# pansanity666/TransHuman

Hardware: AMD Instinct MI355X
Metric: rays/sec (512x512, 64 samples/ray) (higher is better)
Workload: dtype f32 (fp16 hi/lo x3 MFMA emulation)

## Files before the change

### include/transhuman_hip.h

```cpp
#ifndef TRANSHUMAN_HIP_H
#define TRANSHUMAN_HIP_H

#include <stddef.h>
#include <stdint.h>

#ifdef __cplusplus
extern "C" {
#endif

#define TH_ABI_VERSION 12

typedef struct th_ctx th_ctx;
typedef void* th_stream;

int         th_abi_version(void);
const char* th_last_error(void);
int         th_ctx_create(int device, th_ctx** out);
void        th_ctx_destroy(th_ctx* ctx);
size_t      th_sizeof(const char* type_name);

enum { TH_PROF_HULL = 0, TH_PROF_DPARF = 1, TH_PROF_GATHER = 2, TH_PROF_MLP = 3, TH_PROF_COMPOSITE = 4,
       TH_PROF_VIT = 5, TH_PROF_FOLD = 6 , TH_PROF_PHASES = 8 };
int th_profile_enable(th_ctx* ctx, int on);
int th_profile_read(th_ctx* ctx, double* ms_out, int64_t* count_out);
int th_host_wait_read(th_ctx* ctx, double* ms_out);
int th_clock_probe(th_ctx* ctx, int64_t* out_dev , th_stream stream);
int th_fused_cycles(th_ctx* ctx, int64_t* counters_dev);

typedef struct {
    const float* w;
    const float* b;
    int out_f;
    int in_f;
} th_linear;

typedef struct {
    th_linear fc_0, alpha_res_0;
    th_linear key0, val0;
    th_linear key1, val1;
    th_linear fc_1, fc_2, fc_3, alpha_fc;
    th_linear feature_fc, rgb_res_0, view_fc, rgb_res_1, fc_4, rgb_fc;
    th_linear upsample_color;
} th_mlp_weights;

typedef struct {
    const float *ln1_w, *ln1_b, *ln2_w, *ln2_b;
    th_linear qkv, proj, fc1, fc2;
} th_vit_block;

int th_set_mlp_weights(th_ctx* ctx, const th_mlp_weights* w, th_stream stream);
int th_set_mlp_mode(th_ctx* ctx, int mode);
int th_set_fused_waves(th_ctx* ctx, int waves);
int th_set_tok_gather(th_ctx* ctx, int on);
int th_set_tex_rows(th_ctx* ctx, int on);

#define TH_RANGE_SLOTS 8
#define TH_RANGE_FP16_LIMIT 0x7B53u
#define TH_RANGE_FP16_FLOOR 0x2400u
int th_set_vit_mode(th_ctx* ctx, int mode);
int th_range_snapshot(th_ctx* ctx, th_stream stream);
int th_range_read(th_ctx* ctx, int slot, uint32_t* out );
int th_range_last_slot(th_ctx* ctx);
int th_set_chunk_samples(int n);
int th_set_vit_weights(th_ctx* ctx, int depth, int dim, int heads, const th_vit_block* blocks,
                       const float* norm_w, const float* norm_b, th_stream stream);

size_t th_linear_workspace_bytes(int out_f, int in_f);
int th_linear_forward(th_ctx* ctx, const float* A, int lda, int M, const th_linear* lin, int act,
                      float* C, int ldc, void* workspace, size_t workspace_bytes, th_stream stream);

typedef struct {
    const float* pts;
    const float* ray_o;
    const float* ray_d;
    const float* near;
    const float* far;
    const float* t_vals;
    const float* one_minus_t;
    int R, S;
    const float* z_vals;
    const float* sigma_noise;
} th_points;

size_t th_hull_workspace_bytes(int n_verts);
int th_hull_mask(th_ctx* ctx, const th_points* p, const float* verts_world, int n_verts, float thresh,
                 uint8_t* mask_out, int32_t* ray_hit_out, void* workspace, size_t workspace_bytes,
                 th_stream stream);

int th_paint_group(th_ctx* ctx, const float* holder_map_nchw, int V, int C, int H, int W,
                   const float* verts_world, int n_verts, const float* cams, const float* scale_xy,
                   const uint8_t* vizmap, const int32_t* csr_offsets, const int32_t* csr_members,
                   int n_clusters, float* painted_out , float* tokens_out,
                   th_stream stream);
int th_segment_mean_f32(th_ctx* ctx, const float* src, int width, const int32_t* csr_offsets,
                        const int32_t* csr_members, int n_clusters, float* out, th_stream stream);
int th_segment_mean_rot_f64(th_ctx* ctx, const double* blend, const int32_t* csr_offsets,
                            const int32_t* csr_members, int n_clusters, float* rot_out,
                            th_stream stream);

#define TH_MAP_FULL    384
#define TH_MAP_COMPACT 260
#define TH_MAP_SPLIT   256

int th_upsample_concat_nhwc(th_ctx* ctx, const float* img, const float* lat0, const float* lat1,
                            const float* lat2, const int32_t* dims_host, int V, int H, int W,
                            const float* color_w, const float* color_b, float* out_nhwc, th_stream stream);
int th_upsample_concat_split(th_ctx* ctx, const float* img, const float* lat0, const float* lat1, const float* lat2,
                             const int32_t* dims_host, int V, int H, int W, float* out, th_stream stream);
int th_map_box(th_ctx* ctx, const float* verts_a, int na, const float* verts_b, int nb, const float* cams, int V,
               const float* scale_xy, int H, int W, float reach, int32_t* box_out, th_stream stream);
int th_upsample_concat_split_box(th_ctx* ctx, const float* img, const float* lat0, const float* lat1, const float* lat2,
                                 const int32_t* dims_host, int V, int H, int W, float* out, const int32_t* box,
                                 th_stream stream);
size_t th_map_demand_bytes(int V, int H, int W);
int th_upsample_concat_split_demand(th_ctx* ctx, const float* img, const float* lat0, const float* lat1, const float* lat2,
                                    const int32_t* dims_host, int V, int H, int W, float* out, const int32_t* box,
                                    const void* demand, th_stream stream);
size_t th_paint_group_nhwc_workspace_bytes(int V, int n_verts, int C, int out_f);
int th_paint_group_nhwc(th_ctx* ctx, const float* map_nhwc, int V, int H, int W, int C,
                        const float* verts_world, int n_verts, const float* cams, const float* scale_xy,
                        const uint8_t* vizmap, const th_linear* reduction, const th_linear* color_lift,
                        const int32_t* csr_offsets,
                        const int32_t* csr_members, int n_clusters, float* tokens_out, void* workspace,
                        size_t workspace_bytes, th_stream stream);

size_t th_conv_pack_bytes(int cout, int cin, int ks);
int th_conv_pack(th_ctx* ctx, const float* w, int cout, int cin, int ks, void* packed, size_t packed_bytes,
                 float* inv_scale_out, th_stream stream);
int th_conv2d_supported(int cin, int cout, int ks, int stride);
int th_conv2d(th_ctx* ctx, const float* x, int N, int cin, int H, int W, const void* packed, float inv_scale, int cout,
              int ks, int stride, float* y, th_stream stream);

int th_maxpool3x3s2(th_ctx* ctx, const float* x, int planes, int H, int W, float* y, th_stream stream);

size_t th_bn_workspace_bytes(int N, int C, int HW);
// ... 70 lines not shown
size_t th_ssim_workspace_bytes(int h, int w, int c);
int th_ssim(th_ctx* ctx, const float* a, const float* b, int h, int w, int c, int pitch, double* out, void* workspace,
            size_t workspace_bytes, th_stream stream);

size_t th_lpips_pack_bytes(void);
int th_lpips_pack(th_ctx* ctx, const float* const* conv_w , const float* const* conv_b ,
                  const float* const* lin_w , void* packed, size_t bytes, th_stream stream);
size_t th_lpips_workspace_bytes(int n, int h, int w);
int th_lpips(th_ctx* ctx, const float* in0, const float* in1, int n, int h, int w, const void* packed, double* out,
             void* workspace, size_t workspace_bytes, th_stream stream);

size_t th_rasterize_workspace_bytes(int V, int n_verts, int n_faces, int H, int W);
int th_rasterize_mesh(th_ctx* ctx, const float* verts_world, int n_verts, const int32_t* faces, int n_faces, const float* cams,
                      int V, int H, int W, float background, float* depth, int32_t* pix_to_face, void* workspace,
                      size_t workspace_bytes, th_stream stream);
int th_vertex_visibility(th_ctx* ctx, const int32_t* pix_to_face, const int32_t* faces, int n_faces, int n_verts, int V, int H,
                         int W, uint8_t* vis, th_stream stream);
int th_depth_visibility(th_ctx* ctx, const float* verts_world, int n_verts, const float* cams, int V, const float* depthmaps,
                        int H, int W, float det, float* surface_depth, uint8_t* vis_mask, float* relative_depth,
                        th_stream stream);

size_t th_vertex_normals_workspace_bytes(int n_verts, int n_faces);
int th_vertex_normals(th_ctx* ctx, const float* verts, int n_verts, const int32_t* faces, int n_faces, int flip, float* normals,
                      int32_t* status, void* workspace, size_t workspace_bytes, th_stream stream);
int th_shade_mesh(th_ctx* ctx, const float* verts_world, const float* vertex_normals, int n_verts, const int32_t* faces,
                  int n_faces, const float* cams, int V, int H, int W, const int32_t* pix_to_face, const float* light_host ,
                  const float* background_host , float ambient, float diffuse, float specular, int shininess, float* image,
                  th_stream stream);

int th_prep_views(th_ctx* ctx, const uint8_t* img_u8, const uint8_t* msk_u8, int V, int H0, int W0, const float* K ,
                  const float* D , int n, int mask_bkgd, int white_bkgd, const float* lut , float* out_img,
                  uint8_t* out_msk, th_stream stream);
int th_prep_mask(th_ctx* ctx, const uint8_t* a, const uint8_t* b_or_null, int V, int H0, int W0, int border, uint8_t* out,
                 th_stream stream);

typedef struct {
    const double* v_template;
    const double* shapedirs;
    const double* posedirs;
    const double* J_regressor;
    const double* weights;
    const int32_t* parent;
    int n_verts;
} th_smpl_model;
size_t th_smpl_workspace_bytes(int n_verts);
int th_smpl_lbs(th_ctx* ctx, const th_smpl_model* model, const float* pose_aa, const float* rot, const double* beta,
                double* verts, double* joints, double* T, void* workspace, size_t workspace_bytes,
                th_stream stream);

int th_view_embed(th_ctx* ctx, const float* ray_d, int R, int view_res, float* out, th_stream stream);

typedef struct {
    const int32_t* box;
    float          reach;
    const float*   img;
    const float*   lat0;
    const float*   lat1;
    const float*   lat2;
    int32_t        dims[6];
    const void*    demand;
} th_map_source;

typedef struct {
    const float* verts_world;
    int          n_verts;
    const float* Rh;
    const float* Th;
    const float* cams;
    const float* scale_xy;
    const float* pixel_map_nhwc;
    int          V, H, W;
    int          map_channels;
    const float* tokens;
    const float* centres;
    const float* rot;
    int          n_clusters;
    float        hull_thresh;
    int          small_frame_rays;
    const th_map_source* map_source;
    const float* map_fold;
} th_frame;

size_t th_render_workspace_bytes(const th_frame* f, int R, int S);
size_t th_shade_pool_bytes(th_ctx* ctx, const th_frame* f, long long n_valid, int with_pregather);
int th_render_rays(th_ctx* ctx, const th_frame* f, const th_points* rays, float* rgb, float* acc,
                   float* depth, int white_bkgd, void* workspace, size_t workspace_bytes,
                   void* shade_pool, size_t shade_pool_bytes, int64_t* stats_host, th_stream stream);

int th_render_prepass(th_ctx* ctx, const th_frame* f, const th_points* rays, void* workspace,
                      size_t workspace_bytes, th_stream stream);
int th_render_pregather(th_ctx* ctx, const th_frame* f, const th_points* rays, void* workspace,
                        size_t workspace_bytes, void* shade_pool, size_t shade_pool_bytes, th_stream stream);
int th_render_pregrid(th_ctx* ctx, const th_frame* f, const th_points* rays, void* workspace, size_t workspace_bytes,
                      th_stream stream);
int th_render_predemand(th_ctx* ctx, const th_frame* f, const th_points* rays, void* workspace, size_t workspace_bytes,
                        const float* verts_paint, int n_paint, void* demand, size_t demand_bytes, th_stream stream);
int th_render_pregather_early(th_ctx* ctx, const th_frame* f, const th_points* rays, void* workspace,
                              size_t workspace_bytes, void* shade_pool, size_t shade_pool_bytes, th_stream stream);
int th_render_prepass_wait(th_ctx* ctx, const void* workspace, int64_t* counts_host );
int th_render_prepass_cancel(th_ctx* ctx);
int th_render_prepass_drop(th_ctx* ctx, const void* workspace);

size_t th_sigma_grid_workspace_bytes(const th_frame* f, int P);
int th_eval_sigma_grid(th_ctx* ctx, const th_frame* f, const float* pts, int P, float* sigma_out,
                       void* workspace, size_t workspace_bytes, void* shade_pool, size_t shade_pool_bytes,
                       int64_t* stats_host, th_stream stream);

#ifdef __cplusplus
}
#endif
#endif
```

### transhuman_amd/csrc/k_mlp_fused8_kernel.h

```cpp
#pragma once
#include "k_mlp_fused_kernel.h"

typedef float f8_f4 __attribute__((ext_vector_type(4)));
typedef short f8_s4 __attribute__((ext_vector_type(4)));
typedef short f8_s8 __attribute__((ext_vector_type(8)));

#define F8_THREADS 512
#define F8_PART_FLOATS (3 * 8 * 32)
#define F8_PSTR 12
#define F8_MISC_FLOATS (F8_PSTR * 32 + F8_PART_FLOATS + 32 + 8)
#define F8_LDS_BYTES (ABUF_BYTES + MBUF_BYTES + F8_MISC_FLOATS * 4)
static_assert(F8_LDS_BYTES <= 163840, "the 8-wave tile must fit the CU's LDS");

#define F8_MFMA(A, B, C) __builtin_amdgcn_mfma_f32_16x16x32_f16((A), (B), (C), 0, 0, 0)

template <int CT>
__device__ __forceinline__ void f8_load_w(const uint4* __restrict__ wl, int t, uint4 (&w)[CT][2]) {
    const uint4* p = wl + (long long)t * (CT * 2 * 64);
#pragma unroll
    for (int c = 0; c < CT; ++c) {
        w[c][0] = p[(c * 2 + 0) * 64];
        w[c][1] = p[(c * 2 + 1) * 64];
    }
}
#define F8_WSLICE(L, wave, ct) ((L).w + (long long)(wave) * (L).KB * ((ct) * 2 * 64))

template <int NR, int ROWSTEP, bool PERM>
__device__ __forceinline__ void f8_load_x(const char* __restrict__ ahi, const char* __restrict__ alo, int aoff, int t,
                                          h8 (&xh)[NR], h8 (&xl)[NR]) {
    const int ko = (PERM ? 32 : 64) * t;
#pragma unroll
    for (int r = 0; r < NR; ++r) {
        xh[r] = *reinterpret_cast<const h8*>(ahi + r * ROWSTEP + aoff + ko);
        xl[r] = *reinterpret_cast<const h8*>(alo + r * ROWSTEP + aoff + ko);
    }
}
template <bool PERM>
__device__ __forceinline__ int f8_aoff(int lane, int str) {
    const int l = lane & 15, g = lane >> 4;
    return PERM ? l * str + 16 * (g >> 1) + 256 * (g & 1) : l * str + 16 * g;
}

template <int CT, int RT, int NR, int R0, bool FIRST>
__device__ __forceinline__ void f8_mfma_half(const uint4 (&w)[CT][2], const h8 (&xh)[NR], const h8 (&xl)[NR], f8_f4 (&acc)[CT][RT]) {
    const f8_f4 zero = {0.f, 0.f, 0.f, 0.f};
#pragma unroll
    for (int c = 0; c < CT; ++c)
#pragma unroll
        for (int r = 0; r < NR; ++r)
            acc[c][R0 + r] = F8_MFMA(*reinterpret_cast<const h8*>(&w[c][1]), xh[r], FIRST ? zero : acc[c][R0 + r]);
#pragma unroll
    for (int c = 0; c < CT; ++c)
#pragma unroll
        for (int r = 0; r < NR; ++r) acc[c][R0 + r] = F8_MFMA(*reinterpret_cast<const h8*>(&w[c][0]), xl[r], acc[c][R0 + r]);
#pragma unroll
    for (int c = 0; c < CT; ++c)
#pragma unroll
        for (int r = 0; r < NR; ++r) acc[c][R0 + r] = F8_MFMA(*reinterpret_cast<const h8*>(&w[c][0]), xh[r], acc[c][R0 + r]);
}

template <int NMEM, int NMF>
__device__ __forceinline__ void f8_interleave() {
    constexpr int NP = NMEM < NMF ? NMEM : NMF;
#pragma unroll
    for (int q = 0; q < NP; ++q) {
        __builtin_amdgcn_sched_group_barrier(0x008, 1, 0);
        __builtin_amdgcn_sched_group_barrier(0x120, 1, 0);
    }
    if constexpr (NMF > NP) __builtin_amdgcn_sched_group_barrier(0x008, NMF - NP, 0);
    if constexpr (NMEM > NP) __builtin_amdgcn_sched_group_barrier(0x120, NMEM - NP, 0);
    FM_SB();
}

template <int RT, int CT, int ROWSTEP, bool PERM, bool PRE = false>
__device__ __forceinline__ void f8_gemm(const char* __restrict__ ahi, const char* __restrict__ alo, int str,
                                        const uint4* __restrict__ wp, int T, int lane, f8_f4 (&acc)[CT][RT], uint4 (&w)[2][CT][2]) {
    static_assert(RT % 2 == 0, "row tiles come in halves");
    constexpr int NR = RT / 2;
    const uint4* wl = wp + lane;
    const int aoff = f8_aoff<PERM>(lane, str);
    h8 xah[NR], xal[NR], xbh[NR], xbl[NR];
    if (!PRE) f8_load_w<CT>(wl, 0, w[0]);
    f8_load_x<NR, ROWSTEP, PERM>(ahi, alo, aoff, 0, xah, xal);
    FM_SB();
    auto step = [&](auto first, auto par, int t) __attribute__((always_inline)) {
        constexpr bool F = decltype(first)::value;
        constexpr int PB = decltype(par)::value;
        const int tn = t + 1 < T ? t + 1 : T - 1;
        f8_load_x<NR, ROWSTEP, PERM>(ahi + NR * ROWSTEP, alo + NR * ROWSTEP, aoff, t, xbh, xbl);
        f8_load_w<CT>(wl, tn, w[PB ^ 1]);
        f8_mfma_half<CT, RT, NR, 0, F>(w[PB], xah, xal, acc);
        f8_interleave<2 * NR + 2 * CT, 3 * CT * NR>();
        f8_load_x<NR, ROWSTEP, PERM>(ahi, alo, aoff, tn, xah, xal);
        f8_mfma_half<CT, RT, NR, NR, F>(w[PB], xbh, xbl, acc);
        f8_interleave<2 * NR, 3 * CT * NR>();
    };
    step(std::true_type{}, std::integral_constant<int, 0>{}, 0);
    if (T > 1) {
        step(std::false_type{}, std::integral_constant<int, 1>{}, 1);
#pragma unroll 1
        for (int t = 2; t < T; t += 2) {
            step(std::false_type{}, std::integral_constant<int, 0>{}, t);
            step(std::false_type{}, std::integral_constant<int, 1>{}, t + 1);
        }
    }
}

template <int RT, int CT, int ROWSTEP, bool PERM, bool PRE = false>
__device__ __forceinline__ void f8_gemm3(const char* __restrict__ ahi, const char* __restrict__ alo, int str,
                                         const uint4* __restrict__ wp, int T, int lane, f8_f4 (&acc)[CT][RT], uint4 (&w)[2][CT][2]) {
    static_assert(RT % 3 == 0, "row tiles come in thirds");
    constexpr int NR = RT / 3;
    const uint4* wl = wp + lane;
    const int aoff = f8_aoff<PERM>(lane, str);
    h8 xh[2][NR], xl[2][NR];
    if (!PRE) f8_load_w<CT>(wl, 0, w[0]);
    f8_load_x<NR, ROWSTEP, PERM>(ahi, alo, aoff, 0, xh[0], xl[0]);
    FM_SB();
    auto sub = [&](auto first, auto sidx, int t) __attribute__((always_inline)) {
        constexpr int S = decltype(sidx)::value, G = S % 3, PB = S / 3, CUR = S & 1;
        constexpr bool F = decltype(first)::value && S < 3;
        constexpr int GN = (G + 1) % 3;
        const int tt = t + PB;
        const int tx = G == 2 ? (tt + 1 < T ? tt + 1 : T - 1) : tt;
        f8_load_x<NR, ROWSTEP, PERM>(ahi + GN * NR * ROWSTEP, alo + GN * NR * ROWSTEP, aoff, tx, xh[CUR ^ 1], xl[CUR ^ 1]);
        if constexpr (G == 0) f8_load_w<CT>(wl, tt + 1 < T ? tt + 1 : T - 1, w[PB ^ 1]);
        f8_mfma_half<CT, RT, NR, G * NR, F>(w[PB], xh[CUR], xl[CUR], acc);
        f8_interleave<2 * NR + (G == 0 ? 2 * CT : 0), 3 * CT * NR>();
    };
    auto pair = [&](auto first, int t) __attribute__((always_inline)) {
        sub(first, std::integral_constant<int, 0>{}, t); sub(first, std::integral_constant<int, 1>{}, t);
        sub(first, std::integral_constant<int, 2>{}, t); sub(first, std::integral_constant<int, 3>{}, t);
        sub(first, std::integral_constant<int, 4>{}, t); sub(first, std::integral_constant<int, 5>{}, t);
    };
    pair(std::true_type{}, 0);
#pragma unroll 1
    for (int t = 2; t < T; t += 2) pair(std::false_type{}, t);
}
template <int RT, int CT, int ROWSTEP, bool PERM, bool PRE = false>
__device__ __forceinline__ void f8_gemm_rt(const char* __restrict__ ahi, const char* __restrict__ alo, int str,
                                           const uint4* __restrict__ wp, int T, int lane, f8_f4 (&acc)[CT][RT], uint4 (&w)[2][CT][2]) {
    if constexpr (RT % 3 == 0) f8_gemm3<RT, CT, ROWSTEP, PERM, PRE>(ahi, alo, str, wp, T, lane, acc, w);
    else f8_gemm<RT, CT, ROWSTEP, PERM, PRE>(ahi, alo, str, wp, T, lane, acc, w);
}

template <int STR, bool NONNEG = true>
__device__ __forceinline__ void f8_store_h(const f8_f4& t, int row, int col0, char* __restrict__ hi, char* __restrict__ lo, int lane,
                                           unsigned& rm) {
    const int c = col0 + 4 * (lane >> 4);
    uint2 a, b;
    split_pair(t[0], t[1], a.x, b.x);
    split_pair(t[2], t[3], a.y, b.y);
    range_acc<NONNEG>(rm, a.x);
    range_acc<NONNEG>(rm, a.y);
    *reinterpret_cast<uint2*>(hi + row * STR + 2 * c) = a;
    *reinterpret_cast<uint2*>(lo + row * STR + 2 * c) = b;
}
__device__ __forceinline__ f8_f4 f8_finish(const f8_f4& a, const float4& b, float inv_scale, bool relu) {
    const f32x2 sc = {inv_scale, inv_scale};
    f32x2 y01 = __builtin_elementwise_fma((f32x2){a[0], a[1]}, sc, (f32x2){b.x, b.y});
    f32x2 y23 = __builtin_elementwise_fma((f32x2){a[2], a[3]}, sc, (f32x2){b.z, b.w});
    if (relu) {
        y01 = __builtin_elementwise_max(y01, (f32x2){0.f, 0.f});
        y23 = __builtin_elementwise_max(y23, (f32x2){0.f, 0.f});
    }
    return (f8_f4){y01[0], y01[1], y23[0], y23[1]};
}
__device__ __forceinline__ float f8_xor(float v, int lane, int mask) {
    return __builtin_bit_cast(float, __builtin_amdgcn_ds_bpermute((lane ^ mask) << 2, __builtin_bit_cast(int, v)));
}
__device__ __forceinline__ float4 f8_bias(const float* __restrict__ bias, int col0, int lane) {
    return *reinterpret_cast<const float4*>(bias + col0 + 4 * (lane >> 4));
}

template <int RT, int NV, int H, int R0, bool FIRST>
__device__ __forceinline__ void f8_mfma_dual(const uint4 (&r3)[2][2], const uint4 (&ra)[1][2], const h8 (&mh)[1], const h8 (&ml)[1],
                                             const h8 (&xh)[NV], const h8 (&xl)[NV], f8_f4 (&a3)[2][2], f8_f4 (&va)[1][RT]) {
    const f8_f4 zero = {0.f, 0.f, 0.f, 0.f};
#pragma unroll
    for (int t = 0; t < 3; ++t) {
        const int wp = t == 0 ? 1 : 0;
        const bool lo = t == 1;
        const bool first = FIRST && t == 0;
        a3[0][H] = F8_MFMA(*reinterpret_cast<const h8*>(&r3[0][wp]), lo ? ml[0] : mh[0], first ? zero : a3[0][H]);
#pragma unroll
        for (int r = 0; r < NV; ++r) {
            va[0][R0 + r] = F8_MFMA(*reinterpret_cast<const h8*>(&ra[0][wp]), lo ? xl[r] : xh[r], first ? zero : va[0][R0 + r]);
            if (r == 0) a3[1][H] = F8_MFMA(*reinterpret_cast<const h8*>(&r3[1][wp]), lo ? ml[0] : mh[0], first ? zero : a3[1][H]);
        }
    }
}

template <int V>
__global__ __launch_bounds__(F8_THREADS, 2) void mlp_fused8_kernel(FusedParams P_arg) {
#define PK P_arg
    struct F8Dbg { long long* dbg; };
    const F8Dbg P{PK.dbg};
    extern __shared__ __attribute__((aligned(16))) char lds[];
    char* abuf = lds;
    char* mbuf = lds + ABUF_BYTES;
    float* misc = reinterpret_cast<float*>(lds + ABUF_BYTES + MBUF_BYTES);
    float* probs = misc;
    float* part = misc + F8_PSTR * 32;
    float* sig = part + F8_PART_FLOATS;
    int* flag = reinterpret_cast<int*>(sig + 32);

    const int tid = threadIdx.x, lane = tid & 63, wave = tid >> 6;
    const int l15 = lane & 15, g4 = lane >> 4;
    const int tile = (int)((blockIdx.x & 7) * (gridDim.x >> 3) + (blockIdx.x >> 3));
    const int pbase = tile * FM_PTS;
    if (pbase >= PK.P) return;
    const int npts = min(FM_PTS, PK.P - pbase);
    const int fm_dbg_tile = tile;
    const int zoff = 0;
    constexpr int ROWS = 32 * V, RT = 2 * V;
    constexpr int RS256 = 16 * STR256;
    int dbg_i = 1;
    long long dbg_t = 0;
    long long* dbg_keep = reinterpret_cast<long long*>(flag + 2);
    constexpr float inv_v = 1.0f / (float)V;
    unsigned rmax = 0u;
    unsigned seen_s = 0u, seen_p = 0u, seen_n = 0u, seen_i = 0u, seen_4 = 0u;
    char* a256_lo = abuf + ROWS * STR256;

    struct TexPre { unsigned h0, h1; fm_u4 rq; };
    auto tex_fetch = [&]() __attribute__((always_inline)) {
        int tl = tile;
        asm volatile("" : "+s"(tl));
        TexPre t;
        const unsigned* hb = PK.tex_hdr + (long long)tl * 512;
        t.h0 = hb[lane];
        t.h1 = hb[64 + lane];
        t.rq = (fm_u4){0u, 0u, 0u, 0u};
        if (tid < 64 * V) t.rq = *reinterpret_cast<const fm_u4*>(PK.tex_rec + (long long)tl * V * 32 * 8 + tid * 4);
        return t;
    };
    auto fill_tex = [&](const TexPre& pre, auto rgb, auto&& under) __attribute__((always_inline)) {
        constexpr bool RGB = decltype(rgb)::value;
        constexpr int TSTR = 1040, TMAX = 103, NK = (TMAX + 7) / 8, NR = 4 * V;
        static_assert(TMAX * TSTR <= ABUF_BYTES, "a pass of texel rows must fit the operand buffer");
        int wv = __builtin_amdgcn_readfirstlane(wave), tl = tile;
        asm volatile("" : "+s"(wv), "+s"(tl));
        const unsigned* hb = PK.tex_hdr + (long long)tl * 512;
        unsigned h0 = pre.h0, h1 = pre.h1;
        const int npass = __builtin_amdgcn_readfirstlane((int)(h0 >> 16));
        char* recl = reinterpret_cast<char*>(misc);
        static_assert(32 * V * 32 <= (F8_PSTR * 32 + F8_PART_FLOATS) * 4, "row records must fit probs + part");
        unsigned fv[NR][4] = {};
        f32x2 bias_lo = {0.f, 0.f}, bias_hi = {0.f, 0.f};
        if constexpr (!RGB) {
            const float4 b4 = *reinterpret_cast<const float4*>(PK.ar0.bias + 4 * lane);
            bias_lo = (f32x2){b4.x, b4.y};
            bias_hi = (f32x2){b4.z, b4.w};
        }
        for (int p = 0; p < npass; ++p) {
            if (p > 0) {
                FM_SYNCL();
                h0 = hb[p * 128 + lane];
                h1 = hb[p * 128 + 64 + lane];
            }
            const int U = __builtin_amdgcn_readfirstlane((int)(h0 & 0xffffu));
            {
                constexpr int NA = 7, NB = 10;
                const char* mbase = reinterpret_cast<const char*>(RGB ? PK.tex_map2 : PK.tex_map);
                const unsigned loff = (unsigned)lane * 16u;
                const int last = U - 1;
                fm_u4 ta[NA], tb[NB - NA], tc[NK - NB];
#pragma unroll
                for (int k = 0; k < NA; ++k) {
                    const int i = min(wv + 8 * k, last);
                    const unsigned id = (unsigned)__builtin_amdgcn_readlane((int)h0, 8 + i);
                    ta[k] = *reinterpret_cast<const fm_u4*>(mbase + TX_ADDR(id));
                }
                const bool more = U > 8 * NA, most = U > 8 * NB;
                if (more) {
#pragma unroll
// ... 175 lines not shown
            if (u0 > 0) {
                FM_SYNCL();
                if (tid < 2 * 32 * STRVD / 16) reinterpret_cast<uint4*>(wsp_hi)[tid] = make_uint4(zq, zq, zq, zq);
            }
            for (int u = wv; u < nU; u += 8) {
                const int cu = slot_centre(u0 + u);
                const char* g = reinterpret_cast<const char*>(PK.tsplit) + (long long)cu * 1024 + lane * 16;
#pragma unroll
                for (int vw = 0; vw < V; ++vw)
                    __builtin_amdgcn_global_load_lds((fm_gptr)(g + (long long)vw * PK.t_nc * 1024),
                                                     (fm_lptr)(abuf + (vw * 32 + u) * STOK_STR), 16, 0, 0);
            }
            FM_SYNCL();
            if (slot >= u0 && slot < u0 + 32) {
                _Float16 hi, lo;
                split_h(nw, hi, lo);
                *reinterpret_cast<_Float16*>(wsp_hi + ns * STRVD + 2 * (slot - u0)) = hi;
                *reinterpret_cast<_Float16*>(wsp_lo + ns * STRVD + 2 * (slot - u0)) = lo;
            }
            if (u0 == 0) {
#pragma unroll
                for (int t = 0; t < 2; ++t) {
                    h8 xh[2], xl[2];
                    f8_load_x<2, 16 * STR64, false>(pe_hi, pe_lo, aoffp, t, xh, xl);
                    if (t == 0) f8_mfma_half<2, 2, 2, 0, true>(wq[0], xh, xl, a1);
                    else f8_mfma_half<2, 2, 2, 0, false>(wq[1], xh, xl, a1);
                }
            }
            FM_SYNC();
            {
                h8 xh[2], xl[2];
                f8_load_x<2, 16 * STRVD, false>(wsp_hi, wsp_lo, aoffw, 0, xh, xl);
                const int tq = l15 >> 2, tc = 8 * (l15 & 3);
                const int ro0 = min(8 * g4 + tq, nU - 1) * STOK_STR + tc, ro1 = min(8 * g4 + 4 + tq, nU - 1) * STOK_STR + tc;
                typedef __attribute__((address_space(3))) f8_s4* f8_lp;
#pragma unroll
                for (int r = 0; r < V; ++r)
#pragma unroll
                    for (int c = 0; c < 2; ++c) {
                        const char* rb = abuf + r * 32 * STOK_STR + 2 * (wave * 32 + c * 16);
                        const f8_s4 h0 = __builtin_amdgcn_ds_read_tr16_b64_v4i16((f8_lp)(rb + ro0));
                        const f8_s4 h1 = __builtin_amdgcn_ds_read_tr16_b64_v4i16((f8_lp)(rb + ro1));
                        const f8_s4 l0 = __builtin_amdgcn_ds_read_tr16_b64_v4i16((f8_lp)(rb + ro0 + 512));
                        const f8_s4 l1 = __builtin_amdgcn_ds_read_tr16_b64_v4i16((f8_lp)(rb + ro1 + 512));
                        const f8_s8 ahs = __builtin_shufflevector(h0, h1, 0, 1, 2, 3, 4, 5, 6, 7);
                        const f8_s8 als = __builtin_shufflevector(l0, l1, 0, 1, 2, 3, 4, 5, 6, 7);
                        const h8 ah = __builtin_bit_cast(h8, ahs), al = __builtin_bit_cast(h8, als);
#pragma unroll
                        for (int h = 0; h < 2; ++h) {
                            acc2[c][2 * r + h] = F8_MFMA(al, xh[h], acc2[c][2 * r + h]);
                            acc2[c][2 * r + h] = F8_MFMA(ah, xl[h], acc2[c][2 * r + h]);
                            acc2[c][2 * r + h] = F8_MFMA(ah, xh[h], acc2[c][2 * r + h]);
                        }
                    }
            }
        }
        FM_SYNCL();
        {
            asm volatile("" : "+v"(rv4), "+v"(rv1));
            seen_s = (unsigned)__builtin_amdgcn_readfirstlane((int)rv4[0]);
            seen_p = (unsigned)__builtin_amdgcn_readfirstlane((int)rv4[1]);
            seen_n = (unsigned)__builtin_amdgcn_readfirstlane((int)rv4[2]);
            seen_i = (unsigned)__builtin_amdgcn_readfirstlane((int)rv4[3]);
            seen_4 = (unsigned)__builtin_amdgcn_readfirstlane((int)rv1);
        }
#pragma unroll
        for (int c = 0; c < 2; ++c) {
            f8_f4 pe2[2];
#pragma unroll
            for (int h = 0; h < 2; ++h) pe2[h] = f8_finish(a1[c][h], b0[c], PK.fc_0pe.inv_scale, false);
#pragma unroll
            for (int r = 0; r < RT; ++r) {
                const f32x2 it2 = {inv_t, inv_t};
                f32x2 u01 = __builtin_elementwise_fma((f32x2){acc2[c][r][0], acc2[c][r][1]}, it2, (f32x2){pe2[r & 1][0], pe2[r & 1][1]});
                f32x2 u23 = __builtin_elementwise_fma((f32x2){acc2[c][r][2], acc2[c][r][3]}, it2, (f32x2){pe2[r & 1][2], pe2[r & 1][3]});
                u01 = __builtin_elementwise_max(u01, (f32x2){0.f, 0.f});
                u23 = __builtin_elementwise_max(u23, (f32x2){0.f, 0.f});
                const f8_f4 u = {u01[0], u01[1], u23[0], u23[1]};
                f8_store_h<STR256>(u, r * 16 + l15, wave * 32 + c * 16, abuf, a256_lo, lane, rmax);
            }
        }
        range_commit(PK.range, TH_RANGE_S, seen_s, rmax);
    }
    uint4 wk3[2][3][2];
    FM_SB();
    f8_load_w<3>(F8_WSLICE(PK.w16.kv1, wave, 3) + lane, 0, wk3[0]);
    FM_SYNCL();
    f8_f4 vs[2][RT];
    float* ksb = reinterpret_cast<float*>(mbuf);
    {
        f8_f4 acc3[3][RT];
        f8_gemm_rt<RT, 3, RS256, true, true>(abuf, a256_lo, STR256, F8_WSLICE(PK.w16.kv1, wave, 3), 8, lane, acc3, wk3);
        const float4 bk = f8_bias(PK.kv1.bias, wave * 16, lane), bv0 = f8_bias(PK.kv1.bias, 128 + wave * 32, lane),
                     bv1 = f8_bias(PK.kv1.bias, 128 + wave * 32 + 16, lane);
#pragma unroll
        for (int r = 0; r < RT; ++r) {
            const f8_f4 k = f8_finish(acc3[0][r], bk, PK.kv1.inv_scale, false);
            *reinterpret_cast<float4*>(ksb + (r * 16 + l15) * KSTR + wave * 16 + 4 * g4) = make_float4(k[0], k[1], k[2], k[3]);
            vs[0][r] = f8_finish(acc3[1][r], bv0, PK.kv1.inv_scale, false);
            vs[1][r] = f8_finish(acc3[2][r], bv1, PK.kv1.inv_scale, false);
        }
    }
    FM_SYNCL();

    FM_SB();
    fill_tex(tex_pre, std::false_type{}, [] {});
    FM_SB();
    f8_load_w<3>(F8_WSLICE(PK.w16.kv0, wave, 3) + lane, 0, wk3[0]);
    FM_SYNCL();
    f8_f4 vp[2][RT];
    {
        f8_f4 acc3[3][RT];
        f8_gemm_rt<RT, 3, RS256, true, true>(abuf, a256_lo, STR256, F8_WSLICE(PK.w16.kv0, wave, 3), 8, lane, acc3, wk3);
        const float4 bk = f8_bias(PK.kv0.bias, wave * 16, lane), bv0 = f8_bias(PK.kv0.bias, 128 + wave * 32, lane),
                     bv1 = f8_bias(PK.kv0.bias, 128 + wave * 32 + 16, lane);
        FM_SYNCL();
        float* kpb = reinterpret_cast<float*>(abuf);
#pragma unroll
        for (int r = 0; r < RT; ++r) {
            const f8_f4 k = f8_finish(acc3[0][r], bk, PK.kv0.inv_scale, false);
            *reinterpret_cast<float4*>(kpb + (r * 16 + l15) * KSTR + wave * 16 + 4 * g4) = make_float4(k[0], k[1], k[2], k[3]);
            vp[0][r] = f8_finish(acc3[1][r], bv0, PK.kv0.inv_scale, false);
            vp[1][r] = f8_finish(acc3[2][r], bv1, PK.kv0.inv_scale, false);
        }
    }
    FM_SYNCL();

    {
        const float* kpb = reinterpret_cast<const float*>(abuf);
        float4 bn[2];
        {
            const int p = tid >> 4, c16 = tid & 15;
            f32x2 acc2[V * V];
#pragma unroll
            for (int ji = 0; ji < V * V; ++ji) acc2[ji] = (f32x2){0.f, 0.f};
#pragma unroll
            for (int q = 0; q < 2; ++q) {
                float4 kx[V], sx[V];
#pragma unroll
                for (int v = 0; v < V; ++v) {
                    kx[v] = *reinterpret_cast<const float4*>(kpb + (v * 32 + p) * KSTR + 4 * (c16 + 16 * q));
                    sx[v] = *reinterpret_cast<const float4*>(ksb + (v * 32 + p) * KSTR + 4 * (c16 + 16 * q));
                }
#pragma unroll
                for (int j = 0; j < V; ++j)
#pragma unroll
                    for (int i = 0; i < V; ++i) {
                        acc2[j * V + i] = __builtin_elementwise_fma((f32x2){kx[j].x, kx[j].y}, (f32x2){sx[i].x, sx[i].y}, acc2[j * V + i]);
                        acc2[j * V + i] = __builtin_elementwise_fma((f32x2){kx[j].z, kx[j].w}, (f32x2){sx[i].z, sx[i].w}, acc2[j * V + i]);
                    }
            }
            float acc[V * V];
#pragma unroll
            for (int ji = 0; ji < V * V; ++ji) {
                float s = acc2[ji][0] + acc2[ji][1];
                s += __builtin_bit_cast(float, __builtin_amdgcn_update_dpp(0, __builtin_bit_cast(int, s), 0xB1, 0xF, 0xF, true));
                s += __builtin_bit_cast(float, __builtin_amdgcn_update_dpp(0, __builtin_bit_cast(int, s), 0x4E, 0xF, 0xF, true));
                s += __builtin_bit_cast(float, __builtin_amdgcn_update_dpp(0, __builtin_bit_cast(int, s), 0x141, 0xF, 0xF, true));
                s += __builtin_bit_cast(float, __builtin_amdgcn_update_dpp(0, __builtin_bit_cast(int, s), 0x140, 0xF, 0xF, true));
                acc[ji] = s;
            }
            float a[V], m = -3.0e38f;
#pragma unroll
            for (int j = 0; j < V; ++j) {
                float x = acc[j * V];
#pragma unroll
// ... 11 lines not shown
        }
        bn[0] = f8_bias(PK.fc_1.bias, wave * 32, lane);
        bn[1] = f8_bias(PK.fc_1.bias, wave * 32 + 16, lane);
        FM_SYNCL();
#pragma unroll
        for (int h = 0; h < 2; ++h) {
            const float* pr = probs + (h * 16 + l15) * F8_PSTR;
            const float4 q0 = *reinterpret_cast<const float4*>(pr), q1 = *reinterpret_cast<const float4*>(pr + 4);
            const float q2 = pr[8];
            const float A[9] = {q0.x, q0.y, q0.z, q0.w, q1.x, q1.y, q1.z, q1.w, q2};
#pragma unroll
            for (int c = 0; c < 2; ++c) {
                const f32x2 b01 = {bn[c].x, bn[c].y}, b23 = {bn[c].z, bn[c].w};
                f32x2 t0[V], t1[V];
#pragma unroll
                for (int i = 0; i < V; ++i) {
                    t0[i] = (f32x2){vs[c][2 * i + h][0], vs[c][2 * i + h][1]} + b01;
                    t1[i] = (f32x2){vs[c][2 * i + h][2], vs[c][2 * i + h][3]} + b23;
                }
#pragma unroll
                for (int j = 0; j < V; ++j) {
                    const f32x2 v0 = {vp[c][2 * j + h][0], vp[c][2 * j + h][1]}, v1 = {vp[c][2 * j + h][2], vp[c][2 * j + h][3]};
#pragma unroll
                    for (int i = 0; i < V; ++i) {
                        const f32x2 a2 = {A[j * V + i], A[j * V + i]};
                        t0[i] = __builtin_elementwise_fma(v0, a2, t0[i]);
                        t1[i] = __builtin_elementwise_fma(v1, a2, t1[i]);
                    }
                }
#pragma unroll
                for (int i = 0; i < V; ++i) {
                    t0[i] = __builtin_elementwise_max(t0[i], (f32x2){0.f, 0.f});
                    t1[i] = __builtin_elementwise_max(t1[i], (f32x2){0.f, 0.f});
                    const f8_f4 n = {t0[i][0], t0[i][1], t1[i][0], t1[i][1]};
                    f8_store_h<STR256>(n, (2 * i + h) * 16 + l15, wave * 32 + c * 16, abuf, a256_lo, lane, rmax);
                }
            }
        }
        range_commit(PK.range, TH_RANGE_N, seen_n, rmax);
    }

    uint4 wk2[2][2][2];
    FM_SB();
    f8_load_w<2>(F8_WSLICE(PK.w16.fc_2, wave, 2) + lane, 0, wk2[0]);
#pragma unroll
    for (int q = 0; q < 2; ++q) {
        const int i = tid + F8_THREADS * q, row = i >> 5, c = i & 31;
        int x = pbase + row;
        if (PK.vd_sel != nullptr && PK.rgb_all != 2 && c < 27 && row < npts) x = PK.vd_sel[pbase + row];
        vsel[q] = x;
    }
    FM_SYNCL();
    f8_gemm_rt<RT, 2, RS256, true, true>(abuf, a256_lo, STR256, F8_WSLICE(PK.w16.fc_2, wave, 2), 8, lane, acc2, wk2);
    const float4 bi[2] = {f8_bias(PK.fc_2.bias, wave * 32, lane), f8_bias(PK.fc_2.bias, wave * 32 + 16, lane)};
#pragma unroll
    for (int q = 0; q < 2; ++q) {
        const int i = tid + F8_THREADS * q, row = i >> 5, c = i & 31;
        float x = 0.f;
        if (PK.rgb_all != 2 && c < 27 && row < npts) {
            const long long vr = PK.vd_sel ? (long long)(vsel[q] / PK.vd_div) : (long long)(pbase + row);
            x = PK.vd[vr * 27 + c];
        }
        vdv[q] = x;
    }
    FM_SYNCL();
#pragma unroll
    for (int c = 0; c < 2; ++c) {
#pragma unroll
        for (int r = 0; r < RT; ++r) acc2[c][r] = f8_finish(acc2[c][r], bi[c], PK.fc_2.inv_scale, true);
#pragma unroll
        for (int h = 0; h < 2; ++h) {
            f8_f4 m = acc2[c][h];
#pragma unroll
            for (int r = 1; r < V; ++r) m = m + acc2[c][2 * r + h];
            m = m * (f8_f4){inv_v, inv_v, inv_v, inv_v};
            f8_store_h<STR256>(m, h * 16 + l15, wave * 32 + c * 16, mbuf, mbuf + 32 * STR256, lane, rmax);
        }
#pragma unroll
        for (int r = 0; r < RT; ++r) f8_store_h<STR256>(acc2[c][r], r * 16 + l15, wave * 32 + c * 16, abuf, a256_lo, lane, rmax);
    }
    range_commit(PK.range, TH_RANGE_INTER, seen_i, rmax);
    FM_SYNCL();

    char* vd_hi = mbuf + MBUF_VD_OFF;
    char* vd_lo = vd_hi + 32 * STRVD;
    tex_pre2 = tex_fetch();
    f8_f4 va[1][RT];
    {
        f8_f4 a3[2][2];
        const float4 aw[2] = {f8_bias(PK.alpha_w, wave * 32, lane), f8_bias(PK.alpha_w, wave * 32 + 16, lane)};
        const float4 b3[2] = {f8_bias(PK.fc_3.bias, wave * 32, lane), f8_bias(PK.fc_3.bias, wave * 32 + 16, lane)};
        if (PK.rgb_all != 2) {
            constexpr int T = 8;
            const uint4* w3l = F8_WSLICE(PK.w16.fc_3, wave, 2) + lane;
            const uint4* wal = F8_WSLICE(PK.w16.vfA, wave, 1) + lane;
            const int aoff = f8_aoff<true>(lane, STR256);
            const char* mhi = mbuf;
            const char* mlo = mbuf + 32 * STR256;
            uint4 r3[2][2][2], ra[2][1][2];
            h8 mah[1], mal[1], xah[V], xal[V], mbh[1], mbl[1], xbh[V], xbl[V];
            f8_load_w<2>(w3l, 0, r3[0]);
            f8_load_w<1>(wal, 0, ra[0]);
            f8_load_x<1, RS256, true>(mhi, mlo, aoff, 0, mah, mal);
            f8_load_x<V, RS256, true>(abuf, a256_lo, aoff, 0, xah, xal);
            FM_SB();
            auto step = [&](auto first, auto par, int t) __attribute__((always_inline)) {
                constexpr bool F = decltype(first)::value;
                constexpr int PB = decltype(par)::value;
                const int tn = t + 1 < T ? t + 1 : T - 1;
                f8_load_x<1, RS256, true>(mhi + RS256, mlo + RS256, aoff, t, mbh, mbl);
                f8_load_x<V, RS256, true>(abuf + V * RS256, a256_lo + V * RS256, aoff, t, xbh, xbl);
                f8_load_w<2>(w3l, tn, r3[PB ^ 1]);
                f8_load_w<1>(wal, tn, ra[PB ^ 1]);
                f8_mfma_dual<RT, V, 0, 0, F>(r3[PB], ra[PB], mah, mal, xah, xal, a3, va);
                f8_interleave<2 + 2 * V + 6, 3 * (2 + V)>();
                f8_load_x<1, RS256, true>(mhi, mlo, aoff, tn, mah, mal);
                f8_load_x<V, RS256, true>(abuf, a256_lo, aoff, tn, xah, xal);
                f8_mfma_dual<RT, V, 1, V, F>(r3[PB], ra[PB], mbh, mbl, xbh, xbl, a3, va);
                f8_interleave<2 + 2 * V, 3 * (2 + V)>();
            };
            step(std::true_type{}, std::integral_constant<int, 0>{}, 0);
            step(std::false_type{}, std::integral_constant<int, 1>{}, 1);
#pragma unroll 1
            for (int t = 2; t < T; t += 2) {
                step(std::false_type{}, std::integral_constant<int, 0>{}, t);
                step(std::false_type{}, std::integral_constant<int, 1>{}, t + 1);
            }
        } else {
#pragma unroll
            for (int r = 0; r < RT; ++r) va[0][r] = (f8_f4){0.f, 0.f, 0.f, 0.f};
            uint4 w3[2][2][2];
            f8_gemm<2, 2, RS256, true, false>(mbuf, mbuf + 32 * STR256, STR256, F8_WSLICE(PK.w16.fc_3, wave, 2), 8, lane, a3, w3);
        }
        float s2[2];
#pragma unroll
        for (int h = 0; h < 2; ++h) {
            float s = 0.f;
#pragma unroll
            for (int c = 0; c < 2; ++c) {
                const f8_f4 y = f8_finish(a3[c][h], b3[c], PK.fc_3.inv_scale, true);
                s = fmaf(y[0], aw[c].x, s);
                s = fmaf(y[1], aw[c].y, s);
                s = fmaf(y[2], aw[c].z, s);
                s = fmaf(y[3], aw[c].w, s);
            }
            s += f8_xor(s, lane, 16);
            s += f8_xor(s, lane, 32);
            s2[h] = s;
        }
        if (g4 == 0) part[wave * 32 + l15] = s2[0];
        if (g4 == 1) part[wave * 32 + 16 + l15] = s2[1];
        if (tid == 0) *flag = 0;
        FM_SYNCL();
        if (tid < 32) {
            float sg = PK.alpha_b[zoff];
#pragma unroll
            for (int w = 0; w < 8; ++w) sg += part[w * 32 + tid];
            sig[tid] = sg;
            if (tid < npts && PK.rgb_all != 2 && (PK.rgb_all == 1 || sg > 0.f)) *flag = 1;
        }
#pragma unroll
        for (int q = 0; q < 2; ++q) {
            const int i = tid + F8_THREADS * q, row = i >> 5, c = i & 31;
            _Float16 a, b;
            split_h(vdv[q], a, b);
            *reinterpret_cast<_Float16*>(vd_hi + row * STRVD + 2 * c) = a;
            *reinterpret_cast<_Float16*>(vd_lo + row * STRVD + 2 * c) = b;
        }
        FM_SYNCL();
    }
    const bool need_rgb = *flag != 0;
    float rgb_out[3] = {0.f, 0.f, 0.f};
    if (need_rgb) {
        uint4 wvd[1][2];
        f8_load_w<1>(F8_WSLICE(PK.w16.vfD, wave, 1) + lane, 0, wvd);
        FM_SB();
        fill_tex(tex_pre2, std::true_type{}, [&]() __attribute__((always_inline)) {
            h8 xh[2], xl[2];
            f8_load_x<2, 16 * STRVD, false>(vd_hi, vd_lo, f8_aoff<false>(lane, STRVD), 0, xh, xl);
#pragma unroll
            for (int r = 0; r < RT; ++r) {
                va[0][r] = F8_MFMA(*reinterpret_cast<const h8*>(&wvd[0][1]), xh[r & 1], va[0][r]);
                va[0][r] = F8_MFMA(*reinterpret_cast<const h8*>(&wvd[0][0]), xl[r & 1], va[0][r]);
                va[0][r] = F8_MFMA(*reinterpret_cast<const h8*>(&wvd[0][0]), xh[r & 1], va[0][r]);
            }
        });
        FM_SYNCL();
        uint4 w4[4][1][2];
        {
            const uint4* wl4 = F8_WSLICE(PK.w16.fc_4, wave, 1) + lane;
#pragma unroll
            for (int t = 0; t < 4; ++t) f8_load_w<1>(wl4, t, w4[t]);
        }
        float4 rw[3];
#pragma unroll
        for (int o = 0; o < 3; ++o) rw[o] = f8_bias(PK.rgb_w + o * 128, wave * 16, lane);
        const float4 b4 = f8_bias(PK.fc_4.bias, wave * 16, lane);
        const float4 bt = f8_bias(PK.rst.bias, wave * 16, lane), br = f8_bias(PK.rst.bias, 128 + wave * 16, lane);
        char* f4_hi = mbuf + MBUF_FC4_OFF;
        char* f4_lo = f4_hi + 32 * STR128;
        {
            const char* mb = abuf + l15 * 1040 + 4 * (wave * 16 + 4 * g4);
            f8_f4 u[RT];
#pragma unroll
            for (int r = 0; r < RT; ++r) {
                const float4 m1 = *reinterpret_cast<const float4*>(mb + r * 16 * 1040);
                const float4 m2 = *reinterpret_cast<const float4*>(mb + r * 16 * 1040 + 512);
                const f8_f4 t = f8_finish(va[0][r], bt, PK.rst.inv_scale, false);
                const f32x2 z2 = {0.f, 0.f};
                const f32x2 u01 = __builtin_elementwise_max((f32x2){t[0], t[1]} + (f32x2){m1.x, m1.y}, z2) + ((f32x2){m2.x, m2.y} + (f32x2){br.x, br.y});
                const f32x2 u23 = __builtin_elementwise_max((f32x2){t[2], t[3]} + (f32x2){m1.z, m1.w}, z2) + ((f32x2){m2.z, m2.w} + (f32x2){br.z, br.w});
                u[r] = (f8_f4){u01[0], u01[1], u23[0], u23[1]};
            }
#pragma unroll
            for (int h = 0; h < 2; ++h) {
                f8_f4 m = u[h];
#pragma unroll
                for (int r = 1; r < V; ++r) m = m + u[2 * r + h];
                m = m * (f8_f4){inv_v, inv_v, inv_v, inv_v};
                f8_store_h<STR128, false>(m, h * 16 + l15, wave * 16, f4_hi, f4_lo, lane, rmax);
            }
            range_commit(PK.range, TH_RANGE_F4, seen_4, rmax);
        }
        FM_SYNCL();
        f8_f4 a4[1][2];
        {
            const int aoff4 = f8_aoff<false>(lane, STR128);
#pragma unroll
            for (int t = 0; t < 4; ++t) {
                h8 xh4[2], xl4[2];
                f8_load_x<2, 16 * STR128, false>(f4_hi, f4_lo, aoff4, t, xh4, xl4);
                if (t == 0) f8_mfma_half<1, 2, 2, 0, true>(w4[t], xh4, xl4, a4);
                else f8_mfma_half<1, 2, 2, 0, false>(w4[t], xh4, xl4, a4);
            }
        }
        float s3[3][2];
#pragma unroll
        for (int h = 0; h < 2; ++h) {
            const f8_f4 y = f8_finish(a4[0][h], b4, PK.fc_4.inv_scale, true);
#pragma unroll
            for (int o = 0; o < 3; ++o) {
                float s = 0.f;
                s = fmaf(y[0], rw[o].x, s);
                s = fmaf(y[1], rw[o].y, s);
                s = fmaf(y[2], rw[o].z, s);
                s = fmaf(y[3], rw[o].w, s);
                s += f8_xor(s, lane, 16);
                s += f8_xor(s, lane, 32);
                s3[o][h] = s;
            }
        }
#pragma unroll
// ... 24 lines not shown
```

### transhuman_amd/csrc/k_mlp_fused_host.hip

```cpp
#include <stdio.h>
#include <stdlib.h>
#include <string.h>

#include "k_mlp_fused_kernel.h"
#include "k_mlp_fused8_kernel.h"

__global__ void pack_fused_kernel(const float* __restrict__ W, int N, int K, int KB, int CT, const int* __restrict__ cols,
                                  float scale, uint4* __restrict__ out) {
    long long total = 4LL * KB * CT * 2 * 64;
    for (long long o = blockIdx.x * (long long)blockDim.x + threadIdx.x; o < total;
         o += (long long)gridDim.x * blockDim.x) {
        int lane = (int)(o & 63);
        long long q = o >> 6;
        int plane = (int)(q & 1); q >>= 1;
        int ct = (int)(q % CT); q /= CT;
        int kb = (int)(q % KB);
        int wave = (int)(q / KB);
        int col = cols[wave * CT + ct] + (lane & 31);
        int k0 = 16 * kb + 8 * (lane >> 5);
        h8 v;
#pragma unroll
        for (int j = 0; j < 8; ++j) {
            int k = k0 + j;
            float x = (col < N && k < K) ? W[(long long)col * K + k] * scale : 0.f;
// ... 309 lines not shown
    TH_HIP(hipMemsetAsync(amax, 0, 4, s));
    hipLaunchKernelGGL(absmax_kernel, dim3(64), dim3(256), 0, s, tprime, (long long)rows * 256, amax);
    hipLaunchKernelGGL(tok_split_kernel, dim3(th_cdiv(rows, 4) < 1024 ? th_cdiv(rows, 4) : 1024), dim3(256), 0, s, tprime, rows, sc,
                       range);
    TH_LAUNCH_CHECK();
    return 0;
}

int th_map_fold_launch(const FusedParams& base, const float* map_split, int V, int H, int W, const int32_t* box, float* fold,
                       unsigned int* range, hipStream_t s, const unsigned* demand) {
    TH_REQUIRE(base.compact_ready, "the map fold needs the colour-folded layers (th_mlp_weights.upsample_color)");
    TH_REQUIRE(V >= 1 && H >= 1 && W >= 1 && map_split && fold, "bad argument");
    MapFoldParams p;
    p.ar0 = base.ar0c; p.rst = base.rstc;
    p.lat = map_split; p.rgb = map_split + (size_t)V * H * W * 256;
    p.box = box; p.V = V; p.H = H; p.W = W;
    p.out0 = fold; p.out12 = fold + (size_t)V * H * W * 256;
    p.range = range;
    p.list = nullptr; p.count = nullptr;
    static unsigned long long attr_done = 0ull;
    if (th_lds_attr_needed(&attr_done)) {
        TH_HIP(hipFuncSetAttribute((const void*)map_fold_kernel<false>, hipFuncAttributeMaxDynamicSharedMemorySize, 2 * MF_TEX * STR272));
        TH_HIP(hipFuncSetAttribute((const void*)map_fold_kernel<true>, hipFuncAttributeMaxDynamicSharedMemorySize, 2 * MF_TEX * STR272));
    }
    if (demand != nullptr) {
        const size_t NW = (size_t)V * H * W / 32;
        p.count = demand + 2 * NW;
        p.list = reinterpret_cast<const int32_t*>(demand + 2 * NW + 16);
        hipLaunchKernelGGL(map_fold_kernel<true>, dim3(512), dim3(256), 2 * MF_TEX * STR272, s, p);
        TH_LAUNCH_CHECK();
        return 0;
    }
    const int tpr = (W + MF_TEX - 1) / MF_TEX;
    hipLaunchKernelGGL(map_fold_kernel<false>, dim3((unsigned)(V * H * tpr)), dim3(256), 2 * MF_TEX * STR272, s, p);
    TH_LAUNCH_CHECK();
    return 0;
}

int th_mlp_fused_forward(const FusedParams& base, const ThMlpPacked& heads, int V, int P, const float* stok,
                         const void* pe, const void* f, int f_ld, const float* vd, const int32_t* vd_sel, int vd_div, int rgb_all, float* raw_c,
                         unsigned int* range, hipStream_t s, const void* tsplit, const float* t_inv, int t_nc, const float* tex_map,
                         size_t tex_stride) {
    if (P <= 0) return 0;
    TH_REQUIRE(V >= 1 && V <= 3, "fused MLP supports 1..3 reference views");
    TH_REQUIRE(f_ld == 384 || (f_ld == 272 && base.compact_ready),
               "pixel-feature rows must be 384 wide, or 272 wide with upsample_color weights uploaded");
    const bool cf = f_ld == 272;
    FusedParams p = base;
    if (cf) { p.ar0 = base.ar0c; p.rst = base.rstc; }
    p.alpha_w = heads.alpha_w; p.alpha_b = heads.alpha_b; p.rgb_w = heads.rgb_w; p.rgb_b = heads.rgb_b;
    TH_REQUIRE(tsplit == nullptr || (t_inv != nullptr && t_nc >= 7 && t_nc <= 4096), "split token table: scale word and 7 <= N_c <= 4096");
    p.tsplit = (const _Float16*)tsplit; p.t_inv = t_inv; p.t_nc = t_nc;
    const bool tex = tex_map != nullptr;
    TH_REQUIRE(!tex || (cf && f != nullptr), "texel hand-over: compact (272-wide) operand planes only");
    p.tex_hdr = nullptr; p.tex_rec = nullptr; p.tex_map = nullptr; p.tex_map2 = nullptr;
    if (tex) {
        p.tex_hdr = (const unsigned*)f;
        p.tex_rec = p.tex_hdr + (size_t)th_cdiv(P, FM_PTS) * 512;
        p.tex_map = tex_map;
        p.tex_map2 = tex_map + tex_stride;
        f = nullptr;
    }
    p.stok = stok; p.pe = (const _Float16*)pe; p.f = (const _Float16*)f; p.vd = vd; p.vd_sel = vd_sel; p.vd_div = vd_div > 0 ? vd_div : 1; p.raw_c = raw_c; p.P = P; p.rgb_all = rgb_all; p.range = range;
    static unsigned long long attr_done = 0ull;
    if (th_lds_attr_needed(&attr_done)) {
#define FM_ATTR(V_, F_)                                                                                       \
    TH_HIP(hipFuncSetAttribute((const void*)mlp_fused_kernel<V_, F_>, hipFuncAttributeMaxDynamicSharedMemorySize, \
                               FUSED_LDS_BYTES))
        FM_ATTR(1, 0); FM_ATTR(2, 0); FM_ATTR(3, 0); FM_ATTR(1, 1); FM_ATTR(2, 1); FM_ATTR(3, 1);
#undef FM_ATTR
#define FM_ATTR_T(V_)                                                                                              \
    TH_HIP(hipFuncSetAttribute((const void*)mlp_fused_kernel<V_, 1, true>, hipFuncAttributeMaxDynamicSharedMemorySize, \
                               FUSED_LDS_BYTES))
        FM_ATTR_T(1); FM_ATTR_T(2); FM_ATTR_T(3);
#undef FM_ATTR_T
    }
    dim3 grid(tex ? 8 * th_cdiv(th_cdiv(P, FM_PTS), 8) : th_cdiv(P, FM_PTS));
    const bool eight = base.waves == 8 && tex && tsplit != nullptr;
    static unsigned long long attr8_done = 0ull;
    if (eight && th_lds_attr_needed(&attr8_done)) {
        TH_HIP(hipFuncSetAttribute((const void*)mlp_fused8_kernel<1>, hipFuncAttributeMaxDynamicSharedMemorySize, F8_LDS_BYTES));
        TH_HIP(hipFuncSetAttribute((const void*)mlp_fused8_kernel<2>, hipFuncAttributeMaxDynamicSharedMemorySize, F8_LDS_BYTES));
        TH_HIP(hipFuncSetAttribute((const void*)mlp_fused8_kernel<3>, hipFuncAttributeMaxDynamicSharedMemorySize, F8_LDS_BYTES));
    }
    static int dbg_state = getenv("TH_FUSED_DBG") ? 1 : 0;
    static long long* dbg_dev = nullptr;
    p.dbg = base.cycles_buf;
    const bool dbg_now = dbg_state == 1 && P >= 4096 && base.cycles_buf == nullptr;
    hipEvent_t dbg_e0 = nullptr, dbg_e1 = nullptr;
    if (dbg_now) {
        if (!dbg_dev) TH_HIP(hipMalloc((void**)&dbg_dev, 64 * sizeof(long long)));
        TH_HIP(hipMemsetAsync(dbg_dev, 0, 64 * sizeof(long long), s));
        p.dbg = dbg_dev;
        TH_HIP(hipEventCreate(&dbg_e0));
        TH_HIP(hipEventCreate(&dbg_e1));
        TH_HIP(hipStreamSynchronize(s));
        TH_HIP(hipEventRecord(dbg_e0, s));
    }
#define FM_LAUNCH(V_, F_) hipLaunchKernelGGL((mlp_fused_kernel<V_, F_>), grid, dim3(256), FUSED_LDS_BYTES, s, p)
#define FM_LAUNCH_T(V_) hipLaunchKernelGGL((mlp_fused_kernel<V_, 1, true>), grid, dim3(256), FUSED_LDS_BYTES, s, p)
#define FM_LAUNCH_8(V_) hipLaunchKernelGGL((mlp_fused8_kernel<V_>), grid, dim3(F8_THREADS), F8_LDS_BYTES, s, p)
    if (eight) {
        if (V == 1) FM_LAUNCH_8(1); else if (V == 2) FM_LAUNCH_8(2); else FM_LAUNCH_8(3);
    } else if (tex) {
        if (V == 1) FM_LAUNCH_T(1); else if (V == 2) FM_LAUNCH_T(2); else FM_LAUNCH_T(3);
    } else
    switch (V * 2 + (cf ? 1 : 0)) {
        case 2: FM_LAUNCH(1, 0); break;
        case 3: FM_LAUNCH(1, 1); break;
        case 4: FM_LAUNCH(2, 0); break;
        case 5: FM_LAUNCH(2, 1); break;
        case 6: FM_LAUNCH(3, 0); break;
        default: FM_LAUNCH(3, 1); break;
    }
#undef FM_LAUNCH
#undef FM_LAUNCH_T
#undef FM_LAUNCH_8
    TH_LAUNCH_CHECK();
    if (dbg_now) {
        long long st[64];
        TH_HIP(hipEventRecord(dbg_e1, s));
        TH_HIP(hipStreamSynchronize(s));
        float dbg_ms = 0.f;
        TH_HIP(hipEventElapsedTime(&dbg_ms, dbg_e0, dbg_e1));
        fprintf(stderr, "[TH_FUSED_DBG] launch %.3f ms (events), %d tiles\n", dbg_ms, grid.x);
        TH_HIP(hipMemcpy(st, dbg_dev, sizeof(st), hipMemcpyDeviceToHost));
        fprintf(stderr, "[TH_FUSED_DBG] %lld tiles sampled of %d, average cycles between barriers:", st[0], grid.x);
        long long tot = 0;
        for (int i = 1; i < 62 && st[i] != 0; ++i) {
            fprintf(stderr, " %lld", st[i] / (st[0] > 0 ? st[0] : 1));
            tot += st[i] / (st[0] > 0 ? st[0] : 1);
        }
        fprintf(stderr, "  | total %lld", tot);
        if (st[63] > 0)
            fprintf(stderr, "  | %.1f us per tile at %.3f GHz inside the launch", (double)st[63] / (double)(st[0] > 0 ? st[0] : 1) * 0.01,
                    (double)st[62] / ((double)st[63] * 10.0));
        fprintf(stderr, "\n");
        dbg_state = 2;
    }
    return 0;
}
```

### transhuman_amd/csrc/th_api.hip

```cpp
#include <stdlib.h>
#include <string.h>

#include <vector>

#include "th_internal.h"

static thread_local std::string g_err;
void th_set_error(const std::string& msg) { g_err = msg; }

struct ThProf {
    bool on = false;
    std::vector<hipEvent_t> pool;
    size_t used = 0;
    struct Span { int phase; hipEvent_t a, b; };
    std::vector<Span> spans;
    hipEvent_t get() {
        if (used == pool.size()) {
            hipEvent_t e;
            if (hipEventCreate(&e) != hipSuccess) return nullptr;
            pool.push_back(e);
        }
        return pool[used++];
    }
};
struct ProfScope {
    ThProf* p; int phase; hipStream_t s; hipEvent_t a = nullptr;
    ProfScope(ThProf* p_, int phase_, hipStream_t s_) : p(p_), phase(phase_), s(s_) {
        if (p && p->on) {
            hipStreamCaptureStatus st = hipStreamCaptureStatusNone;
            if (hipStreamIsCapturing(s, &st) != hipSuccess || st != hipStreamCaptureStatusNone) return;
            a = p->get();
            if (a) (void)hipEventRecord(a, s);
        }
    }
    void close() {
        if (a) { hipEvent_t b = p->get(); if (b) { (void)hipEventRecord(b, s); p->spans.push_back({phase, a, b}); } }
        a = nullptr;
    }
    ~ProfScope() { close(); }
};
static ThProf* prof_of(th_ctx* c);
__global__ void clock_probe_kernel(long long* __restrict__ out, int iters) {
    float x = 1.0f + threadIdx.x * 1e-3f;
    const long long t0 = clock64(), w0 = wall_clock64();
    for (int i = 0; i < iters; ++i) x = fmaf(x, 0.999f, 1e-3f);
    const long long t1 = clock64(), w1 = wall_clock64();
    if (threadIdx.x == 0) { out[0] = t1 - t0; out[1] = w1 - w0; }
    if (x == 12345.678f) out[2] = 1;
}


extern "C" {

int th_abi_version(void) { return TH_ABI_VERSION; }
const char* th_last_error(void) { return g_err.c_str(); }
size_t th_sizeof(const char* type_name) {
    if (type_name == nullptr) return 0;
#define TH_SZ(T) if (strcmp(type_name, #T) == 0) return sizeof(T)
    TH_SZ(th_points); TH_SZ(th_frame); TH_SZ(th_map_source); TH_SZ(th_linear); TH_SZ(th_mlp_weights); TH_SZ(th_vit_block); TH_SZ(th_smpl_model);
#undef TH_SZ
    return 0;
}

int th_ctx_create(int device, th_ctx** out) {
    TH_REQUIRE(out != nullptr, "null out");
    int count = 0;
    TH_HIP(hipGetDeviceCount(&count));
    TH_REQUIRE(device >= 0 && device < count, "no such device");
    TH_HIP(hipSetDevice(device));
    hipDeviceProp_t prop;
    TH_HIP(hipGetDeviceProperties(&prop, device));
    TH_REQUIRE(std::string(prop.gcnArchName).rfind("gfx950", 0) == 0,
               std::string("libtranshuman_hip is built for gfx950 only, device is ") + prop.gcnArchName);
    th_ctx* c = new th_ctx();
    c->device = device;
    c->n_cu = prop.multiProcessorCount;
    if (const char* e = getenv("TH_TOK_GATHER")) c->tok_gather = e[0] == '0' ? 0 : 1;
    if (const char* e = getenv("TH_ROWS_TEX")) c->tex_rows = e[0] == '0' ? 0 : 1;
    c->fused.waves = 8;
    if (const char* e = getenv("TH_FUSED_WAVES")) c->fused.waves = e[0] == '4' ? 4 : 8;
    TH_HIP(hipHostMalloc((void**)&c->host_pinned, 64 * sizeof(int32_t), hipHostMallocDefault));
    TH_HIP(hipMalloc((void**)&c->range_dev, TH_RANGE_SLOTS * sizeof(unsigned int)));
    TH_HIP(hipMemset(c->range_dev, 0, TH_RANGE_SLOTS * sizeof(unsigned int)));
    TH_HIP(hipHostMalloc((void**)&c->range_host, th_ctx::kRangeSnaps * TH_RANGE_SLOTS * sizeof(unsigned int),
                         hipHostMallocDefault));
    memset(c->range_host, 0, th_ctx::kRangeSnaps * TH_RANGE_SLOTS * sizeof(unsigned int));
    *out = c;
    return 0;
}

void th_ctx_destroy(th_ctx* c) {
    if (!c) return;
    if (c->mlp_store) (void)hipFree(c->mlp_store);
    if (c->vit_store) (void)hipFree(c->vit_store);
    if (c->fused_store) (void)hipFree(c->fused_store);
    if (c->host_pinned) (void)hipHostFree(c->host_pinned);
    if (c->range_dev) (void)hipFree(c->range_dev);
    if (c->range_host) (void)hipHostFree(c->range_host);
    if (c->aux) (void)hipStreamDestroy(c->aux);
    if (c->aux2) (void)hipStreamDestroy(c->aux2);
    if (c->aux2_join) (void)hipEventDestroy(c->aux2_join);
    if (c->aux_fork) (void)hipEventDestroy(c->aux_fork);
    if (c->aux_join) (void)hipEventDestroy(c->aux_join);
    if (c->after_shade) (void)hipEventDestroy(c->after_shade);
    for (auto& e : c->range_ev)
        if (e) (void)hipEventDestroy(e);
    for (auto& t : c->prepass)
        if (t.ev) (void)hipEventDestroy(t.ev);
    delete[] c->vit.blocks;
    if (c->prof) {
        ThProf* p = (ThProf*)c->prof;
        for (auto e : p->pool) (void)hipEventDestroy(e);
        delete p;
    }
    delete c;
}

int th_profile_enable(th_ctx* c, int on) {
    TH_REQUIRE(c, "null ctx");
    ThProf* p = prof_of(c);
    p->on = on != 0;
    p->used = 0;
    p->spans.clear();
    return 0;
}

int th_clock_probe(th_ctx* c, int64_t* out_dev, th_stream stream) {
    TH_REQUIRE(c && out_dev, "null argument");
    hipLaunchKernelGGL(clock_probe_kernel, dim3(1), dim3(64), 0, (hipStream_t)stream, (long long*)out_dev, 4096);
    TH_LAUNCH_CHECK();
    return 0;
}

int th_fused_cycles(th_ctx* c, int64_t* counters_dev) {
    TH_REQUIRE(c, "null ctx");
    c->fused.cycles_buf = (long long*)counters_dev;
    return 0;
}

int th_host_wait_read(th_ctx* c, double* ms_out) {
    TH_REQUIRE(c && ms_out, "null argument");
    *ms_out = c->host_wait_ms;
    c->host_wait_ms = 0.0;
    return 0;
}

int th_profile_read(th_ctx* c, double* ms_out, int64_t* count_out) {
    TH_REQUIRE(c && ms_out && count_out, "null argument");
    ThProf* p = prof_of(c);
    for (int i = 0; i < TH_PROF_PHASES; ++i) { ms_out[i] = 0.0; count_out[i] = 0; }
    for (auto& sp : p->spans) {
        TH_HIP(hipEventSynchronize(sp.b));
        float ms = 0.f;
        TH_HIP(hipEventElapsedTime(&ms, sp.a, sp.b));
        if (sp.phase >= 0 && sp.phase < TH_PROF_PHASES) { ms_out[sp.phase] += ms; count_out[sp.phase] += 1; }
    }
    p->used = 0;
    p->spans.clear();
    return 0;
}

static bool lin_ok(const th_linear& l, int out_f, int in_f) {
    return l.w != nullptr && l.out_f == out_f && l.in_f == in_f;
// ... 82 lines not shown
            float* fw = (float*)(base + cfold_off + i * th_align((size_t)(256 * 260 + 256) * sizeof(float)));
            float* fb = fw + 256 * 260;
            const int N = src3[i]->out_f;
            TH_TRY(th_fold_color_launch(src3[i]->w, src3[i]->b, w->upsample_color.w, w->upsample_color.b, N, fw, fb, s));
            folded[i].w = fw; folded[i].b = fb; folded[i].out_f = N; folded[i].in_f = 260;
            TH_TRY(th_pack_linear(folded[i], base + po, dst3[i], s));
            po += ThPacked::bytes(N, 260);
        }
        M.compact_ready = true;
    }
    TH_HIP(hipMemsetAsync(c->range_dev + TH_RANGE_CONV, 0, sizeof(unsigned int), s));
    TH_HIP(hipStreamSynchronize(s));
    M.ready = true;
    c->fused_ready = false;
    if (c->fused_store) { TH_HIP(hipFree(c->fused_store)); c->fused_store = nullptr; }
    TH_HIP(hipMalloc(&c->fused_store, th_fused_pack_bytes()));
    TH_TRY(th_fused_pack(w, have_lift ? folded : nullptr, c->fused_store, &c->fused, s));
    c->fused_ready = true;
    return 0;
}

int th_range_snapshot(th_ctx* c, th_stream stream) {
    TH_REQUIRE(c, "null ctx");
    hipStream_t s = (hipStream_t)stream;
    const int gen = c->range_gen_next;
    const int slot = gen % th_ctx::kRangeSnaps;
    c->range_gen_next = gen == 0x3fffffff ? 0 : gen + 1;
    if (!c->range_ev[slot]) TH_HIP(hipEventCreateWithFlags(&c->range_ev[slot], hipEventDisableTiming));
    TH_HIP(hipMemcpyAsync(c->range_host + slot * TH_RANGE_SLOTS, c->range_dev, TH_RANGE_SLOTS * sizeof(unsigned int),
                          hipMemcpyDeviceToHost, s));
    TH_HIP(hipMemsetAsync(c->range_dev, 0, TH_RANGE_CONV * sizeof(unsigned int), s));
    TH_HIP(hipEventRecord(c->range_ev[slot], s));
    c->range_gen[slot] = gen;
    c->range_last = gen;
    return gen;
}

int th_range_read(th_ctx* c, int id, uint32_t* out) {
    TH_REQUIRE(c && out, "null argument");
    TH_REQUIRE(id >= 0, "no such range snapshot");
    const int slot = id % th_ctx::kRangeSnaps;
    TH_REQUIRE(c->range_ev[slot], "no such range snapshot");
    if (c->range_gen[slot] != id) {
        th_set_error("th_range_read: snapshot " + std::to_string(id) + " has been overwritten by later snapshots");
        return 2;
    }
    {
        ThWaitClock wc(c);
        TH_HIP(hipEventSynchronize(c->range_ev[slot]));
    }
    memcpy(out, c->range_host + slot * TH_RANGE_SLOTS, TH_RANGE_SLOTS * sizeof(unsigned int));
    return 0;
}

int th_range_last_slot(th_ctx* c) { return c ? c->range_last : -1; }

int th_set_vit_mode(th_ctx* c, int mode) {
    TH_REQUIRE(c && (mode == 0 || mode == 1), "mode must be 0 (fp32 MFMA GEMMs) or 1 (fp16-split MFMA GEMMs)");
    c->vit_mode = mode;
    return 0;
}

int th_set_tok_gather(th_ctx* c, int on) {
    TH_REQUIRE(c && (on == 0 || on == 1), "th_set_tok_gather: 0 (blended rows from K4) or 1 (neighbour records, blend in the fused kernel)");
    c->tok_gather = on;
    return 0;
}

int th_set_tex_rows(th_ctx* c, int on) {
    TH_REQUIRE(c && (on == 0 || on == 1), "th_set_tex_rows: 0 (pixel-feature rows from K5) or 1 (texel lists, blend in the fused kernel)");
    c->tex_rows = on;
    return 0;
}

int th_set_mlp_mode(th_ctx* c, int mode) {
    TH_REQUIRE(c && (mode == 0 || mode == 1), "mode must be 0 (layer-by-layer fp32 MFMA) or 1 (fused fp16-split MFMA)");
    c->mlp_mode = mode;
    return 0;
}

int th_set_fused_waves(th_ctx* c, int waves) {
    TH_REQUIRE(c && (waves == 4 || waves == 8), "th_set_fused_waves: 4 (one wave per SIMD) or 8 (two per SIMD)");
    c->fused.waves = waves;
    return 0;
}

int th_set_vit_weights(th_ctx* c, int depth, int dim, int heads, const th_vit_block* blocks, const float* norm_w,
                       const float* norm_b, th_stream stream) {
    TH_REQUIRE(c && blocks && norm_w && norm_b, "null argument");
    TH_REQUIRE(depth > 0 && dim == heads * 64, "ViT must have head_dim 64");
    hipStream_t s = (hipStream_t)stream;
    size_t per = ThPacked::bytes(3 * dim, dim) + ThPacked::bytes(dim, dim) + ThPacked::bytes(4 * dim, dim) +
                 ThPacked::bytes(dim, 4 * dim) + th_align(4 * dim * sizeof(float)) +
                 ThPacked::bytes_h3(3 * dim, dim) + ThPacked::bytes_h3(dim, dim) + ThPacked::bytes_h3(4 * dim, dim) +
                 ThPacked::bytes_h3(dim, 4 * dim);
    size_t total = per * depth + th_align(2 * dim * sizeof(float));
    if (c->vit_store) { TH_HIP(hipFree(c->vit_store)); c->vit_store = nullptr; }
    TH_HIP(hipMalloc(&c->vit_store, total));
    delete[] c->vit.blocks;
    c->vit.blocks = new ThVitBlockPacked[depth];
    c->vit.depth = depth; c->vit.dim = dim; c->vit.heads = heads;
    char* base = (char*)c->vit_store;
    size_t off = 0;
    for (int b = 0; b < depth; ++b) {
        const th_vit_block& B = blocks[b];
        ThVitBlockPacked& P = c->vit.blocks[b];
        TH_REQUIRE(lin_ok(B.qkv, 3 * dim, dim) && lin_ok(B.proj, dim, dim) && lin_ok(B.fc1, 4 * dim, dim) &&
                       lin_ok(B.fc2, dim, 4 * dim) && B.ln1_w && B.ln1_b && B.ln2_w && B.ln2_b,
                   "unexpected ViT block shape");
        TH_TRY(th_pack_linear(B.qkv, base + off, &P.qkv, s)); off += ThPacked::bytes(3 * dim, dim);
        TH_TRY(th_pack_linear(B.proj, base + off, &P.proj, s)); off += ThPacked::bytes(dim, dim);
        TH_TRY(th_pack_linear(B.fc1, base + off, &P.fc1, s)); off += ThPacked::bytes(4 * dim, dim);
        TH_TRY(th_pack_linear(B.fc2, base + off, &P.fc2, s)); off += ThPacked::bytes(dim, 4 * dim);
        TH_TRY(th_pack_linear_h3(B.qkv, base + off, &P.qkv, s)); off += ThPacked::bytes_h3(3 * dim, dim);
        TH_TRY(th_pack_linear_h3(B.proj, base + off, &P.proj, s)); off += ThPacked::bytes_h3(dim, dim);
        TH_TRY(th_pack_linear_h3(B.fc1, base + off, &P.fc1, s)); off += ThPacked::bytes_h3(4 * dim, dim);
        TH_TRY(th_pack_linear_h3(B.fc2, base + off, &P.fc2, s)); off += ThPacked::bytes_h3(dim, 4 * dim);
        float* ln = (float*)(base + off); off += th_align(4 * dim * sizeof(float));
        P.ln1_w = ln; P.ln1_b = ln + dim; P.ln2_w = ln + 2 * dim; P.ln2_b = ln + 3 * dim;
        TH_HIP(hipMemcpyAsync(P.ln1_w, B.ln1_w, dim * 4, hipMemcpyDeviceToDevice, s));
        TH_HIP(hipMemcpyAsync(P.ln1_b, B.ln1_b, dim * 4, hipMemcpyDeviceToDevice, s));
        TH_HIP(hipMemcpyAsync(P.ln2_w, B.ln2_w, dim * 4, hipMemcpyDeviceToDevice, s));
        TH_HIP(hipMemcpyAsync(P.ln2_b, B.ln2_b, dim * 4, hipMemcpyDeviceToDevice, s));
    }
    float* nf = (float*)(base + off);
    c->vit.norm_w = nf; c->vit.norm_b = nf + dim;
    TH_HIP(hipMemcpyAsync(c->vit.norm_w, norm_w, dim * 4, hipMemcpyDeviceToDevice, s));
    TH_HIP(hipMemcpyAsync(c->vit.norm_b, norm_b, dim * 4, hipMemcpyDeviceToDevice, s));
    TH_HIP(hipMemsetAsync(c->range_dev + TH_RANGE_VIT, 0, sizeof(unsigned int), s));
    TH_HIP(hipStreamSynchronize(s));
    c->vit.ready = true;
    return 0;
}

size_t th_linear_workspace_bytes(int out_f, int in_f) { return ThPacked::bytes(out_f, in_f); }

int th_linear_forward(th_ctx* c, const float* A, int lda, int M, const th_linear* lin, int act, float* C, int ldc,
                      void* ws, size_t ws_bytes, th_stream stream) {
    TH_REQUIRE(c && A && lin && C && ws, "null argument");
    TH_REQUIRE(ws_bytes >= ThPacked::bytes(lin->out_f, lin->in_f), "workspace too small");
    TH_REQUIRE(act >= 0 && act <= 2, "act must be 0 (none), 1 (relu) or 2 (gelu)");
    ThPacked P;
    TH_TRY(th_pack_linear(*lin, ws, &P, (hipStream_t)stream));
    return th_gemm(A, lda, M, P, act, C, ldc, (hipStream_t)stream);
}

size_t th_hull_workspace_bytes(int n_verts) { return th_hull_ws(n_verts); }

int th_hull_mask(th_ctx* c, const th_points* p, const float* verts, int nv, float thresh, uint8_t* mask,
                 int32_t* ray_hit, void* ws, size_t ws_bytes, th_stream stream) {
    TH_REQUIRE(c && p && verts && mask && ws, "null argument");
    TH_REQUIRE(p->pts || (p->ray_o && p->ray_d && p->near && p->far && p->t_vals && p->one_minus_t),
               "need explicit pts or a complete ray description");
    ThPointSrc ps = th_src(p);
    long long P = (long long)p->R * p->S;
    return th_hull_mask_launch(ps, P, verts, nv, thresh, mask, ray_hit, ws, ws_bytes, (hipStream_t)stream);
}

int th_paint_group(th_ctx* c, const float* map, int V, int C, int H, int W, const float* verts, int nv,
                   const float* cams, const float* scale, const uint8_t* viz, const int32_t* off, const int32_t* mem,
                   int nc, float* painted, float* tokens, th_stream stream) {
    TH_REQUIRE(c && map && verts && cams && scale && off && mem && tokens, "null argument");
    TH_REQUIRE(painted != nullptr, "painted_out scratch [V,n_verts,C] is required");
    hipStream_t s = (hipStream_t)stream;
    TH_TRY(th_paint_launch(map, V, C, H, W, verts, nv, cams, scale, viz, painted, s));
    return th_segmean_launch(painted, V, (long long)nv * C, C, off, mem, nc, tokens, s);
// ... 760 lines not shown
            const hipError_t e4 = e3 == hipSuccess ? hipStreamWaitEvent(s, c->aux2_join, 0) : e3;
            if (e4 != hipSuccess) (void)hipStreamSynchronize(c->aux2);
        }
        if (rc != 0) return rc;
        if (!t.ev2) TH_HIP(hipEventCreateWithFlags(&t.ev2, hipEventDisableTiming));
        TH_HIP(hipEventRecord(t.ev2, s));
        t.npre = m;
        t.pre_map = f->pixel_map_nhwc;
        t.pre_centres = f->centres;
        t.pre_pool = pool;
        return 0;
    }
    int npre = 0;
    if (prepass == 2) {
        th_ctx::Prepass& t = c->prepass[slot];
        if (t.npre > 0 && can_pre && t.pre_map == f->pixel_map_nhwc && t.pre_centres == f->centres && t.pre_pool == pool) {
            npre = t.npre;
            TH_HIP(hipStreamWaitEvent(s, t.ev2, 0));
        }
        t.npre = 0;
    }
    const PoolPlan pl = pool_plan(c, V, f_ld, n, npre > 0, tex);
    TH_REQUIRE(n <= 0 || (pool != nullptr && pool_bytes >= pl.total), "shading pool too small (th_shade_pool_bytes)");
    TH_REQUIRE(npre == 0 || npre == pl.pre_n, "pre-gather stage and shading disagree on the pool layout");
    ChunkBufs cb{};
    const int CH = pl.ch;
    cb.raw_c = (float*)(pb + pl.raw_c);
    if (CH > 0) {
        cb.h = (float*)(pb + pl.b_h); cb.f = (float*)(pb + pl.b_f); cb.vdc = (float*)(pb + pl.b_vdc);
        cb.pe = (float*)(pb + pl.b_pe); cb.mlp_ws = pb + pl.b_mlp; cb.mlp_ws_bytes = pl.b_mlp_bytes;
    }
    if (!ray_mode && CH > 0) TH_HIP(hipMemsetAsync(cb.vdc, 0, (size_t)CH * 27 * 4, s));
    TH_REQUIRE(f->n_clusters <= TH_MAX_CLUSTERS, "too many token clusters");
    const float* table = nullptr;
    if (n > 0) {
        if (npre > 0 && c->prepass[slot].pre_tokens == f->tokens && mlp_is_fused(c, V)) table = tprime;
        else TH_TRY(token_table(c, f->tokens, V, f->n_clusters, tprime, &table, s));
    }
    if (prepass == 2) c->prepass[slot].pre_tokens = nullptr;
    const bool use_grid = n > npre && getenv("TH_DPARF_NOGRID") == nullptr && th_dparf_grid_ok(f->n_clusters);
    if (use_grid) TH_TRY(th_dparf_grid_build(f->centres, f->n_clusters, gws, gws_b, s));
    if (npre > 0) {
        ChunkBufs pc = cb;
        pc.f = (float*)(pb + pl.a_f); pc.h = (float*)(pb + pl.a_h); pc.pe = (float*)(pb + pl.a_pe);
        {
            ProfScope ps3(pf, TH_PROF_MLP, s);
            TH_TRY(mlp_dispatch(c, V, npre, pc, f_ld, vd_all, idx, S, unmasked, s, tprime, f->n_clusters, tex_map, tex_stride));
        }
        ProfScope ps4(pf, TH_PROF_COMPOSITE, s);
        TH_TRY(th_scatter_raw_launch(cb.raw_c, idx, npre, unmasked, raw, s));
    }
    for (int o = npre; o < n; o += CH) {
        int m = (n - o) < CH ? (n - o) : CH;
        const int32_t* sel = idx + o;
        {
            ProfScope ps2(pf, TH_PROF_GATHER, s);
            if (tex) TH_TRY(th_pixtex_launch(V, f->H, f->W, &ps, sel, m, f->cams, f->scale_xy, cb.f, s));
            else TH_TRY(th_pixgather_launch(f->pixel_map_nhwc, V, f->map_channels, f->H, f->W, nullptr, &ps, sel, m, f->cams,
                                            f->scale_xy, cb.f, f_ld, fmt, s, c->range_dev));
        }
        {
            ProfScope ps1(pf, TH_PROF_DPARF, s);
            TH_TRY(th_dparf_launch(nullptr, &ps, f->Rh, f->Th, sel, m, f->centres, f->rot, table, V,
                                   f->n_clusters, 0.5f, cb.h, cb.pe, dparf_row_format(c, V), use_grid ? gws : nullptr, s));
        }
        {
            ProfScope ps3(pf, TH_PROF_MLP, s);
            if (ray_mode) TH_TRY(mlp_dispatch(c, V, m, cb, f_ld, vd_all, sel, S, unmasked, s, tprime, f->n_clusters, tex_map, tex_stride));
            else TH_TRY(mlp_dispatch(c, V, m, cb, f_ld, cb.vdc, nullptr, 1, 2, s, tprime, f->n_clusters, tex_map, tex_stride));
        }
        ProfScope ps4(pf, TH_PROF_COMPOSITE, s);
        TH_TRY(th_scatter_raw_launch(cb.raw_c, sel, m, unmasked, raw, s));
    }
    *raw_out = raw;
    *mask_out = mask;
    if (ray_hit_out) *ray_hit_out = ray_mode ? ray_hit : nullptr;
    return 0;
}

size_t th_render_workspace_bytes(const th_frame* f, int R, int S) {
    return shade_ws_bytes(f, (long long)R * S, R);
}

size_t th_shade_pool_bytes(th_ctx* c, const th_frame* f, long long n_valid, int with_pregather) {
    if (!c || !f || f->V < 1) return 0;
    const int f_ld = frame_f_ld(f);
    const bool tex = tex_rows(c, f);
    size_t a = pool_plan(c, f->V, f_ld, n_valid, false, tex).total;
    if (with_pregather) {
        const size_t b = pool_plan(c, f->V, f_ld, n_valid, true, tex).total;
        if (b > a) a = b;
    }
    return a;
}

int th_render_prepass_wait(th_ctx* c, const void* ws, int64_t* counts_host) {
    TH_REQUIRE(c && ws && counts_host, "null argument");
    for (int k = 0; k < th_ctx::kPrepassSlots; ++k) {
        th_ctx::Prepass& t = c->prepass[k];
        if (!t.valid || t.ws != ws || !t.ev) continue;
        {
            ThWaitClock wc(c);
            TH_HIP(hipEventSynchronize(t.ev));
        }
        const int32_t* hp = c->host_pinned + 16 + 4 * k;
        counts_host[0] = hp[0]; counts_host[1] = hp[1]; counts_host[2] = hp[2];
        return 0;
    }
    return 1;
}

int th_render_rays(th_ctx* c, const th_frame* f, const th_points* rays, float* rgb, float* acc, float* depth,
                   int white_bkgd, void* ws, size_t ws_bytes, void* pool, size_t pool_bytes, int64_t* stats_host,
                   th_stream stream) {
    TH_REQUIRE(c && f && rays && rgb && acc && depth && ws, "null argument");
    TH_TRY(frame_ok(f));
    TH_REQUIRE(rays->pts == nullptr && rays->ray_o && rays->ray_d && rays->near && rays->far && rays->t_vals &&
                   rays->one_minus_t,
               "th_render_rays needs a complete ray description");
    hipStream_t s = (hipStream_t)stream;
    const int R = rays->R, S = rays->S;
    if (R <= 0) return 0;
    long long P = (long long)R * S;
    TH_REQUIRE(P < (1LL << 31), "R*S must fit in int32");
    TH_REQUIRE(ws_bytes >= shade_ws_bytes(f, P, R), "workspace too small");
    ThArena ar(ws, ws_bytes);
    ThPointSrc ps = th_src(rays);
    float* raw = nullptr;
    const uint8_t* mask = nullptr;
    int slot = -1;
    for (int k = 0; k < th_ctx::kPrepassSlots; ++k) {
        th_ctx::Prepass& t = c->prepass[k];
        if (!t.valid || t.ws != ws) continue;
        t.valid = false;
        if (t.rays == (const void*)rays->ray_o && t.R == R && t.S == S) slot = k;
    }
    const int32_t* ray_hit = nullptr;
    TH_TRY(shade_points(c, f, ps, P, true, ar, pool, pool_bytes, &raw, &mask, stats_host, s, slot >= 0 ? 2 : 0,
                        slot >= 0 ? slot : 0, &ray_hit));
    if (!c->after_shade) TH_HIP(hipEventCreateWithFlags(&c->after_shade, hipEventDisableTiming));
    TH_HIP(hipEventRecord(c->after_shade, s));
    c->after_shade_stream = s;
    c->after_shade_pool = pool;
    c->after_shade_valid = true;
    ProfScope sc(prof_of(c), TH_PROF_COMPOSITE, s);
    TH_TRY(th_composite_launch(raw, nullptr, ps, white_bkgd, rgb, acc, depth, nullptr, mask, s, ray_hit));
    const int snap = th_range_snapshot(c, stream);
    TH_REQUIRE(snap >= 0, "range snapshot failed");
    if (stats_host) stats_host[2] = snap;
    return 0;
}

int th_render_prepass(th_ctx* c, const th_frame* f, const th_points* rays, void* ws, size_t ws_bytes, th_stream stream) {
    TH_REQUIRE(c && f && rays && ws, "null argument");
    TH_REQUIRE(f->verts_world && f->n_verts > 0 && f->V >= 1 && f->V <= 4, "prepass needs verts_world, n_verts and V");
    TH_REQUIRE(rays->pts == nullptr && rays->ray_o && rays->ray_d && rays->near && rays->far && rays->t_vals &&
                   rays->one_minus_t,
               "th_render_prepass needs a complete ray description");
    hipStream_t s = (hipStream_t)stream;
    const int R = rays->R, S = rays->S;
    int slot = -1;
    for (int k = 0; k < th_ctx::kPrepassSlots && slot < 0; ++k)
        if (c->prepass[k].ws == ws) slot = k;
    for (int k = 0; k < th_ctx::kPrepassSlots && slot < 0; ++k)
        if (!c->prepass[k].valid) slot = k;
    if (slot < 0) slot = c->prepass_rr = (c->prepass_rr + 1) % th_ctx::kPrepassSlots;
// ... 151 lines not shown
```

### transhuman_amd/csrc/th_internal.h

```cpp
#pragma once
#include <hip/hip_runtime.h>
#include <stdint.h>
#include <stddef.h>
#include <time.h>
#include <string>

#include "transhuman_hip.h"

#define TH_WAVE 64

void th_set_error(const std::string& msg);
#define TH_FAIL(msg)                                                                \
    do {                                                                            \
        th_set_error(std::string(__func__) + ": " + (msg));                         \
        return -1;                                                                  \
    } while (0)
#define TH_REQUIRE(cond, msg)                                                       \
    do {                                                                            \
        if (!(cond)) TH_FAIL(msg);                                                  \
    } while (0)
#define TH_HIP(call)                                                                \
    do {                                                                            \
        hipError_t e__ = (call);                                                    \
        if (e__ != hipSuccess) {                                                    \
// ... 111 lines not shown
        float t = th_sample_z(ps, ray, s);
        x = ps.ray_o[3 * ray] + ps.ray_d[3 * ray] * t;
        y = ps.ray_o[3 * ray + 1] + ps.ray_d[3 * ray + 1] * t;
        z = ps.ray_o[3 * ray + 2] + ps.ray_d[3 * ray + 2] * t;
    }
}

struct Bilin {
    int i00, i01, i10, i11;
    float w00, w01, w10, w11;
    int x0, y0, x1, y1;
};

__device__ __forceinline__ Bilin th_bilinear_setup(float u, float v, float sx, float sy, int H, int W) {
    float gx = u * sx - 1.0f, gy = v * sy - 1.0f;
    float ix = ((gx + 1.0f) / 2.0f) * (float)(W - 1);
    float iy = ((gy + 1.0f) / 2.0f) * (float)(H - 1);
    ix = fminf(fmaxf(ix, 0.0f), (float)(W - 1));
    iy = fminf(fmaxf(iy, 0.0f), (float)(H - 1));
    float x0 = floorf(ix), y0 = floorf(iy);
    float x1 = x0 + 1.0f, y1 = y0 + 1.0f;
    Bilin b;
    b.w00 = (x1 - ix) * (y1 - iy);
    b.w01 = (ix - x0) * (y1 - iy);
    b.w10 = (x1 - ix) * (iy - y0);
    b.w11 = (ix - x0) * (iy - y0);
    int xi0 = (int)x0, yi0 = (int)y0, xi1 = xi0 + 1, yi1 = yi0 + 1;
    bool bx1 = xi1 <= W - 1, by1 = yi1 <= H - 1;
    if (!bx1) { b.w01 = 0.f; b.w11 = 0.f; xi1 = W - 1; }
    if (!by1) { b.w10 = 0.f; b.w11 = 0.f; yi1 = H - 1; }
    b.i00 = yi0 * W + xi0; b.i01 = yi0 * W + xi1; b.i10 = yi1 * W + xi0; b.i11 = yi1 * W + xi1;
    b.x0 = xi0; b.y0 = yi0; b.x1 = xi1; b.y1 = yi1;
    return b;
}

__device__ __forceinline__ void th_project(const float* __restrict__ cam, float x, float y, float z, float& u,
                                           float& v) {
    float cx = fmaf(cam[2], z, fmaf(cam[1], y, cam[0] * x)) + cam[9];
    float cy = fmaf(cam[5], z, fmaf(cam[4], y, cam[3] * x)) + cam[10];
    float cz = fmaf(cam[8], z, fmaf(cam[7], y, cam[6] * x)) + cam[11];
    const float* K = cam + 12;
    float px = fmaf(K[2], cz, fmaf(K[1], cy, K[0] * cx));
    float py = fmaf(K[5], cz, fmaf(K[4], cy, K[3] * cx));
    float pz = fmaf(K[8], cz, fmaf(K[7], cy, K[6] * cx));
    u = px / pz;
    v = py / pz;
}

#endif

struct ThMlpPacked {
    ThPacked fc_0, alpha_res_0, kv0, kv1, fc_1, fc_2, fc_3, feature_fc, rgb_res_0, view_fc, rgb_res_1, fc_4;
    ThPacked fc_0tok;
    ThPacked alpha_res_0c, rgb_res_0c, rgb_res_1c;
    bool compact_ready = false;
    float *alpha_w = nullptr, *alpha_b = nullptr;
    float *rgb_w = nullptr, *rgb_b = nullptr;
    bool ready = false;
};
struct ThVitBlockPacked {
    float *ln1_w, *ln1_b, *ln2_w, *ln2_b;
    ThPacked qkv, proj, fc1, fc2;
};
struct ThVitPacked {
    int depth = 0, dim = 0, heads = 0;
    ThVitBlockPacked* blocks = nullptr;
    float *norm_w = nullptr, *norm_b = nullptr;
    bool ready = false;
};

struct FusedLayer {
    const uint4* w;
    const float* bias;
    float inv_scale;
    int CT, KB;
    float inv_scale2;
};
struct Fused16 {
    FusedLayer fc_0pe, kv1, kv0, fc_2, fc_3, fc_4, vfA, vfD;
};
struct FusedParams {
    Fused16 w16;
    int waves;
    FusedLayer fc_0pe;
    FusedLayer kv1, ar0, kv0, fc_1, fc_2, fc_3, fc_4;
    FusedLayer vfA, vfD, rst;
    FusedLayer ar0c, rstc;
    bool compact_ready;
    const float *alpha_w, *alpha_b, *rgb_w, *rgb_b;
    const float* stok;
    const _Float16* tsplit;
    const float* t_inv;
    int t_nc;
    const _Float16* pe;
    const _Float16* f;
    const unsigned* tex_hdr;
    const unsigned* tex_rec;
    const float* tex_map;
    const float* tex_map2;
    const float* vd;
    const int32_t* vd_sel;
    int vd_div;
    float* raw_c;
    int P;
    int rgb_all;
    unsigned int* range;
    long long* dbg;
    long long* cycles_buf;
};
enum { TH_RANGE_F = 0, TH_RANGE_S = 1, TH_RANGE_P = 2, TH_RANGE_N = 3, TH_RANGE_INTER = 4, TH_RANGE_F4 = 5, TH_RANGE_CONV = 6,
       TH_RANGE_VIT = 7 };
size_t th_fused_pack_bytes();
int th_fused_pack(const th_mlp_weights* w, const th_linear* folded, void* store, FusedParams* out, hipStream_t s);
int th_mlp_fused_forward(const FusedParams& base, const ThMlpPacked& heads, int V, int P, const float* stok,
                         const void* pe, const void* f, int f_ld, const float* vd, const int32_t* vd_sel, int vd_div, int rgb_all,
                         float* raw_c, unsigned int* range, hipStream_t s, const void* tsplit = nullptr,
                         const float* t_inv = nullptr, int t_nc = 0, const float* tex_map = nullptr, size_t tex_stride = 0);
static inline bool th_lds_attr_needed(unsigned long long* done) {
    int dev = 0;
    if (hipGetDevice(&dev) != hipSuccess || dev < 0 || dev > 63) return true;
    if ((*done >> dev) & 1ull) return false;
    *done |= 1ull << dev;
    return true;
}
int th_map_fold_launch(const FusedParams& base, const float* map_split, int V, int H, int W, const int32_t* box, float* fold,
                       unsigned int* range, hipStream_t s, const unsigned* demand = nullptr );
size_t th_pixtex_bytes(int V, long long P);
int th_pixtex_launch(int V, int H, int W, const ThPointSrc* ps, const int32_t* sel, int P, const float* cams,
                     const float* scale, void* out, hipStream_t s);
int th_tok_split(float* tprime, int rows, float* sc, unsigned int* range, hipStream_t s);

struct th_ctx {
    void* fused_store = nullptr;
    FusedParams fused{};
    bool fused_ready = false;
    int mlp_mode = 1;
    int vit_mode = 1;
    int tok_gather = 1;
    int tex_rows = 1;
    int device = 0;
    void* mlp_store = nullptr;
    void* vit_store = nullptr;
    ThMlpPacked mlp;
    ThVitPacked vit;
    int32_t* host_pinned = nullptr;
    struct Prepass {
        hipEvent_t ev = nullptr;
        const void* ws = nullptr;
        const void* rays = nullptr;
        int R = 0, S = 0;
        bool valid = false;
        hipEvent_t ev2 = nullptr;
        int npre = 0;
        const void* pre_map = nullptr;
        const void* pre_centres = nullptr;
        const void* pre_pool = nullptr;
        const void* grid_centres = nullptr;
        const void* pre_tokens = nullptr;
        const void* demand = nullptr;
        const void* map_done = nullptr;
    };
    static constexpr int kPrepassSlots = 4;
    Prepass prepass[kPrepassSlots];
    int prepass_rr = 0;
    int n_cu = 256;
    const void* map_completed = nullptr;
// ... 142 lines not shown
```

### transhuman_amd/hip.py

```python
import ctypes as C
import os

import torch

_HERE = os.path.dirname(os.path.abspath(__file__))
LIB_PATH = os.environ.get("TH_LIB_PATH") or os.path.join(_HERE, "libtranshuman_hip.so")

c_float_p = C.POINTER(C.c_float)


class ThLinear(C.Structure):
    _fields_ = [("w", C.c_void_p), ("b", C.c_void_p), ("out_f", C.c_int), ("in_f", C.c_int)]


class ThMlpWeights(C.Structure):
    _names = ["fc_0", "alpha_res_0", "key0", "val0", "key1", "val1", "fc_1", "fc_2", "fc_3", "alpha_fc",
              "feature_fc", "rgb_res_0", "view_fc", "rgb_res_1", "fc_4", "rgb_fc", "upsample_color"]
    _fields_ = [(n, ThLinear) for n in _names]


class ThSmplModel(C.Structure):
    _fields_ = [("v_template", C.c_void_p), ("shapedirs", C.c_void_p), ("posedirs", C.c_void_p),
                ("J_regressor", C.c_void_p), ("weights", C.c_void_p), ("parent", C.c_void_p), ("n_verts", C.c_int)]


class ThVitBlock(C.Structure):
    _fields_ = [("ln1_w", C.c_void_p), ("ln1_b", C.c_void_p), ("ln2_w", C.c_void_p), ("ln2_b", C.c_void_p),
                ("qkv", ThLinear), ("proj", ThLinear), ("fc1", ThLinear), ("fc2", ThLinear)]


class ThPoints(C.Structure):
    _fields_ = [("pts", C.c_void_p), ("ray_o", C.c_void_p), ("ray_d", C.c_void_p), ("near", C.c_void_p),
                ("far", C.c_void_p), ("t_vals", C.c_void_p), ("one_minus_t", C.c_void_p), ("R", C.c_int),
                ("S", C.c_int), ("z_vals", C.c_void_p), ("sigma_noise", C.c_void_p)]


class ThFrame(C.Structure):
    _fields_ = [("verts_world", C.c_void_p), ("n_verts", C.c_int), ("Rh", C.c_void_p), ("Th", C.c_void_p),
                ("cams", C.c_void_p), ("scale_xy", C.c_void_p), ("pixel_map_nhwc", C.c_void_p), ("V", C.c_int),
                ("H", C.c_int), ("W", C.c_int), ("map_channels", C.c_int), ("tokens", C.c_void_p), ("centres", C.c_void_p),
                ("rot", C.c_void_p), ("n_clusters", C.c_int), ("hull_thresh", C.c_float),
                ("small_frame_rays", C.c_int), ("map_source", C.c_void_p), ("map_fold", C.c_void_p)]


class ThMapSource(C.Structure):
    _fields_ = [("box", C.c_void_p), ("reach", C.c_float), ("img", C.c_void_p), ("lat0", C.c_void_p),
                ("lat1", C.c_void_p), ("lat2", C.c_void_p), ("dims", C.c_int32 * 6), ("demand", C.c_void_p)]


SYMBOLS = {
    "th_abi_version": (C.c_int, []),
    "th_last_error": (C.c_char_p, []),
    "th_sizeof": (C.c_size_t, [C.c_char_p]),
    "th_ctx_create": (C.c_int, [C.c_int, C.POINTER(C.c_void_p)]),
    "th_ctx_destroy": (None, [C.c_void_p]),
    "th_profile_enable": (C.c_int, [C.c_void_p, C.c_int]),
    "th_profile_read": (C.c_int, [C.c_void_p, C.POINTER(C.c_double), C.POINTER(C.c_int64)]),
    "th_fused_cycles": (C.c_int, [C.c_void_p, C.c_void_p]),
    "th_host_wait_read": (C.c_int, [C.c_void_p, C.POINTER(C.c_double)]),
    "th_clock_probe": (C.c_int, [C.c_void_p, C.c_void_p, C.c_void_p]),
    "th_set_mlp_weights": (C.c_int, [C.c_void_p, C.POINTER(ThMlpWeights), C.c_void_p]),
    "th_set_mlp_mode": (C.c_int, [C.c_void_p, C.c_int]),
    "th_set_fused_waves": (C.c_int, [C.c_void_p, C.c_int]),
    "th_set_vit_mode": (C.c_int, [C.c_void_p, C.c_int]),
    "th_set_tok_gather": (C.c_int, [C.c_void_p, C.c_int]),
    "th_set_tex_rows": (C.c_int, [C.c_void_p, C.c_int]),
    "th_map_fold": (C.c_int, [C.c_void_p, C.c_void_p, C.c_int, C.c_int, C.c_int, C.c_void_p, C.c_void_p, C.c_void_p]),
    "th_pixel_texlist_bytes": (C.c_size_t, [C.c_int, C.c_int]),
    "th_pixel_texlist": (C.c_int, [C.c_void_p, C.c_void_p, C.c_int, C.c_int, C.c_int, C.c_void_p, C.c_void_p, C.c_int,
                                   C.c_void_p, C.c_void_p, C.c_void_p, C.c_size_t, C.c_void_p]),
    "th_range_snapshot": (C.c_int, [C.c_void_p, C.c_void_p]),
    "th_range_read": (C.c_int, [C.c_void_p, C.c_int, C.POINTER(C.c_uint32)]),
    "th_range_last_slot": (C.c_int, [C.c_void_p]),
    "th_set_chunk_samples": (C.c_int, [C.c_int]),
    "th_set_vit_weights": (C.c_int, [C.c_void_p, C.c_int, C.c_int, C.c_int, C.POINTER(ThVitBlock), C.c_void_p,
                                     C.c_void_p, C.c_void_p]),
    "th_linear_workspace_bytes": (C.c_size_t, [C.c_int, C.c_int]),
    "th_linear_forward": (C.c_int, [C.c_void_p, C.c_void_p, C.c_int, C.c_int, C.POINTER(ThLinear), C.c_int,
                                    C.c_void_p, C.c_int, C.c_void_p, C.c_size_t, C.c_void_p]),
    "th_hull_workspace_bytes": (C.c_size_t, [C.c_int]),
    "th_hull_mask": (C.c_int, [C.c_void_p, C.POINTER(ThPoints), C.c_void_p, C.c_int, C.c_float, C.c_void_p,
                               C.c_void_p, C.c_void_p, C.c_size_t, C.c_void_p]),
    "th_paint_group": (C.c_int, [C.c_void_p, C.c_void_p, C.c_int, C.c_int, C.c_int, C.c_int, C.c_void_p, C.c_int,
                                 C.c_void_p, C.c_void_p, C.c_void_p, C.c_void_p, C.c_void_p, C.c_int, C.c_void_p,
                                 C.c_void_p, C.c_void_p]),
    "th_segment_mean_f32": (C.c_int, [C.c_void_p, C.c_void_p, C.c_int, C.c_void_p, C.c_void_p, C.c_int, C.c_void_p,
                                      C.c_void_p]),
    "th_segment_mean_rot_f64": (C.c_int, [C.c_void_p, C.c_void_p, C.c_void_p, C.c_void_p, C.c_int, C.c_void_p,
                                          C.c_void_p]),
    "th_upsample_concat_nhwc": (C.c_int, [C.c_void_p, C.c_void_p, C.c_void_p, C.c_void_p, C.c_void_p,
                                          C.POINTER(C.c_int32), C.c_int, C.c_int, C.c_int, C.c_void_p, C.c_void_p,
                                          C.c_void_p, C.c_void_p]),
    "th_upsample_concat_split": (C.c_int, [C.c_void_p, C.c_void_p, C.c_void_p, C.c_void_p, C.c_void_p,
                                           C.POINTER(C.c_int32), C.c_int, C.c_int, C.c_int, C.c_void_p, C.c_void_p]),
    "th_upsample_concat_split_box": (C.c_int, [C.c_void_p, C.c_void_p, C.c_void_p, C.c_void_p, C.c_void_p,
                                               C.POINTER(C.c_int32), C.c_int, C.c_int, C.c_int, C.c_void_p, C.c_void_p,
                                               C.c_void_p]),
    "th_map_demand_bytes": (C.c_size_t, [C.c_int, C.c_int, C.c_int]),
    "th_upsample_concat_split_demand": (C.c_int, [C.c_void_p, C.c_void_p, C.c_void_p, C.c_void_p, C.c_void_p,
                                                  C.POINTER(C.c_int32), C.c_int, C.c_int, C.c_int, C.c_void_p, C.c_void_p,
                                                  C.c_void_p, C.c_void_p]),
    "th_map_fold_demand": (C.c_int, [C.c_void_p, C.c_void_p, C.c_int, C.c_int, C.c_int, C.c_void_p, C.c_void_p, C.c_void_p]),
    "th_render_predemand": (C.c_int, [C.c_void_p, C.POINTER(ThFrame), C.POINTER(ThPoints), C.c_void_p, C.c_size_t, C.c_void_p,
                                      C.c_int, C.c_void_p, C.c_size_t, C.c_void_p]),
    "th_map_box": (C.c_int, [C.c_void_p, C.c_void_p, C.c_int, C.c_void_p, C.c_int, C.c_void_p, C.c_int, C.c_void_p,
                             C.c_int, C.c_int, C.c_float, C.c_void_p, C.c_void_p]),
    "th_paint_group_nhwc_workspace_bytes": (C.c_size_t, [C.c_int, C.c_int, C.c_int, C.c_int]),
    "th_paint_group_nhwc": (C.c_int, [C.c_void_p, C.c_void_p, C.c_int, C.c_int, C.c_int, C.c_int, C.c_void_p, C.c_int,
                                      C.c_void_p, C.c_void_p, C.c_void_p, C.POINTER(ThLinear), C.POINTER(ThLinear),
                                      C.c_void_p, C.c_void_p, C.c_int, C.c_void_p, C.c_void_p, C.c_size_t, C.c_void_p]),
    "th_vit_workspace_bytes": (C.c_size_t, [C.c_int, C.c_int, C.c_int, C.c_int]),
    "th_vit_forward": (C.c_int, [C.c_void_p, C.c_void_p, C.c_void_p, C.c_int, C.c_int, C.c_void_p, C.c_void_p,
                                 C.c_size_t, C.c_void_p]),
    "th_dparf_encode": (C.c_int, [C.c_void_p, C.c_void_p, C.c_void_p, C.c_int, C.c_void_p, C.c_void_p, C.c_void_p,
                                  C.c_int, C.c_int, C.c_void_p, C.c_void_p]),
    "th_nchw_to_nhwc": (C.c_int, [C.c_void_p, C.c_void_p, C.c_int, C.c_int, C.c_int, C.c_int, C.c_void_p,
                                  C.c_void_p]),
    "th_pixel_gather": (C.c_int, [C.c_void_p, C.c_void_p, C.c_int, C.c_int, C.c_int, C.c_int, C.c_void_p,
                                  C.c_void_p, C.c_int, C.c_void_p, C.c_void_p, C.c_void_p, C.c_int, C.c_void_p]),
    "th_pixel_gather_split": (C.c_int, [C.c_void_p, C.c_void_p, C.c_int, C.c_int, C.c_int, C.c_void_p, C.c_void_p, C.c_int,
                                        C.c_void_p, C.c_void_p, C.c_void_p, C.c_int, C.c_void_p]),
    "th_network_workspace_bytes": (C.c_size_t, [C.c_int, C.c_int]),
    "th_network_forward": (C.c_int, [C.c_void_p, C.c_void_p, C.c_void_p, C.c_void_p, C.c_void_p, C.c_int, C.c_void_p,
                                     C.c_void_p, C.c_void_p, C.c_int, C.c_int, C.c_void_p, C.c_void_p, C.c_size_t,
                                     C.c_void_p]),
    "th_dparf_encode_bwd_workspace_bytes": (C.c_size_t, [C.c_int, C.c_int, C.c_int]),
    "th_dparf_encode_bwd": (C.c_int, [C.c_void_p, C.c_void_p, C.c_int, C.c_void_p, C.c_void_p, C.c_int, C.c_int, C.c_void_p,
                                      C.c_void_p, C.c_void_p, C.c_size_t, C.c_void_p]),
    "th_pixel_gather_bwd": (C.c_int, [C.c_void_p, C.c_int, C.c_int, C.c_int, C.c_int, C.c_void_p, C.c_int, C.c_void_p,
                                      C.c_void_p, C.c_void_p, C.c_int, C.c_void_p, C.c_void_p]),
    "th_composite_bwd": (C.c_int, [C.c_void_p, C.c_void_p, C.c_void_p, C.POINTER(ThPoints), C.c_int, C.c_void_p, C.c_void_p,
                                   C.c_void_p, C.c_void_p, C.c_void_p]),
    "th_composite": (C.c_int, [C.c_void_p, C.c_void_p, C.c_void_p, C.POINTER(ThPoints), C.c_int, C.c_void_p,
                               C.c_void_p, C.c_void_p, C.c_void_p, C.c_void_p]),
    "th_gen_rays": (C.c_int, [C.c_void_p, c_float_p, c_float_p, c_float_p, c_float_p, C.c_int, C.c_int, C.c_void_p,
                              C.c_void_p, C.c_void_p, C.c_void_p, C.c_void_p, C.c_void_p]),
    "th_bound_mask": (C.c_int, [C.c_void_p, C.POINTER(C.c_int32), C.c_int, C.c_int, C.c_void_p, C.c_void_p]),
    "th_ssim_workspace_bytes": (C.c_size_t, [C.c_int, C.c_int, C.c_int]),
    "th_ssim": (C.c_int, [C.c_void_p, C.c_void_p, C.c_void_p, C.c_int, C.c_int, C.c_int, C.c_int, C.c_void_p, C.c_void_p,
                          C.c_size_t, C.c_void_p]),
    "th_rasterize_workspace_bytes": (C.c_size_t, [C.c_int] * 5),
    "th_rasterize_mesh": (C.c_int, [C.c_void_p, C.c_void_p, C.c_int, C.c_void_p, C.c_int, C.c_void_p, C.c_int, C.c_int, C.c_int,
                                    C.c_float, C.c_void_p, C.c_void_p, C.c_void_p, C.c_size_t, C.c_void_p]),
    "th_vertex_visibility": (C.c_int, [C.c_void_p, C.c_void_p, C.c_void_p, C.c_int, C.c_int, C.c_int, C.c_int, C.c_int,
                                       C.c_void_p, C.c_void_p]),
    "th_depth_visibility": (C.c_int, [C.c_void_p, C.c_void_p, C.c_int, C.c_void_p, C.c_int, C.c_void_p, C.c_int, C.c_int,
                                      C.c_float, C.c_void_p, C.c_void_p, C.c_void_p, C.c_void_p]),
    "th_vertex_normals_workspace_bytes": (C.c_size_t, [C.c_int, C.c_int]),
    "th_vertex_normals": (C.c_int, [C.c_void_p, C.c_void_p, C.c_int, C.c_void_p, C.c_int, C.c_int, C.c_void_p, C.c_void_p,
                                    C.c_void_p, C.c_size_t, C.c_void_p]),
    "th_shade_mesh": (C.c_int, [C.c_void_p, C.c_void_p, C.c_void_p, C.c_int, C.c_void_p, C.c_int, C.c_void_p, C.c_int, C.c_int,
                                C.c_int, C.c_void_p, C.POINTER(C.c_float), C.POINTER(C.c_float), C.c_float, C.c_float, C.c_float,
                                C.c_int, C.c_void_p, C.c_void_p]),
    "th_prep_views": (C.c_int, [C.c_void_p, C.c_void_p, C.c_void_p, C.c_int, C.c_int, C.c_int, C.c_void_p, C.c_void_p, C.c_int,
                                C.c_int, C.c_int, C.c_void_p, C.c_void_p, C.c_void_p, C.c_void_p]),
    "th_prep_mask": (C.c_int, [C.c_void_p, C.c_void_p, C.c_void_p, C.c_int, C.c_int, C.c_int, C.c_int, C.c_void_p, C.c_void_p]),
    "th_lpips_pack_bytes": (C.c_size_t, []),
    "th_lpips_pack": (C.c_int, [C.c_void_p, C.c_void_p, C.c_void_p, C.c_void_p, C.c_void_p, C.c_size_t, C.c_void_p]),
    "th_lpips_workspace_bytes": (C.c_size_t, [C.c_int, C.c_int, C.c_int]),
    "th_lpips": (C.c_int, [C.c_void_p, C.c_void_p, C.c_void_p, C.c_int, C.c_int, C.c_int, C.c_void_p, C.c_void_p,
                           C.c_void_p, C.c_size_t, C.c_void_p]),
    "th_marching_cubes_workspace_bytes": (C.c_size_t, [C.c_int, C.c_int, C.c_int]),
    "th_marching_cubes_count": (C.c_int, [C.c_void_p, C.c_void_p, C.c_int, C.c_int, C.c_int, C.c_float, C.c_void_p,
                                          C.c_size_t, C.POINTER(C.c_int64), C.c_void_p]),
    "th_marching_cubes_range": (C.c_int, [C.c_void_p, C.c_void_p, C.c_int, C.c_int, C.c_int, C.c_int,
                                          C.POINTER(C.c_int64), C.c_void_p]),
    "th_marching_cubes_emit": (C.c_int, [C.c_void_p, C.c_void_p, C.c_int, C.c_int, C.c_int, C.c_float, C.c_void_p,
                                         C.c_int, C.c_int, C.POINTER(C.c_double), C.POINTER(C.c_double), C.c_void_p,
                                         C.c_void_p, C.c_void_p]),
    "th_smpl_workspace_bytes": (C.c_size_t, [C.c_int]),
    "th_smpl_lbs": (C.c_int, [C.c_void_p, C.POINTER(ThSmplModel), C.c_void_p, C.c_void_p, C.c_void_p, C.c_void_p,
                              C.c_void_p, C.c_void_p, C.c_void_p, C.c_size_t, C.c_void_p]),
    "th_view_embed": (C.c_int, [C.c_void_p, C.c_void_p, C.c_int, C.c_int, C.c_void_p, C.c_void_p]),
    "th_render_workspace_bytes": (C.c_size_t, [C.POINTER(ThFrame), C.c_int, C.c_int]),
    "th_shade_pool_bytes": (C.c_size_t, [C.c_void_p, C.POINTER(ThFrame), C.c_longlong, C.c_int]),
    "th_render_prepass_wait": (C.c_int, [C.c_void_p, C.c_void_p, C.POINTER(C.c_int64)]),
    "th_render_rays": (C.c_int, [C.c_void_p, C.POINTER(ThFrame), C.POINTER(ThPoints), C.c_void_p, C.c_void_p,
                                 C.c_void_p, C.c_int, C.c_void_p, C.c_size_t, C.c_void_p, C.c_size_t,
                                 C.POINTER(C.c_int64), C.c_void_p]),
    "th_render_prepass": (C.c_int, [C.c_void_p, C.POINTER(ThFrame), C.POINTER(ThPoints), C.c_void_p, C.c_size_t,
                                    C.c_void_p]),
    "th_render_pregrid": (C.c_int, [C.c_void_p, C.POINTER(ThFrame), C.POINTER(ThPoints), C.c_void_p, C.c_size_t,
                                    C.c_void_p]),
    "th_render_pregather": (C.c_int, [C.c_void_p, C.POINTER(ThFrame), C.POINTER(ThPoints), C.c_void_p, C.c_size_t,
                                      C.c_void_p, C.c_size_t, C.c_void_p]),
    "th_render_pregather_early": (C.c_int, [C.c_void_p, C.POINTER(ThFrame), C.POINTER(ThPoints), C.c_void_p, C.c_size_t,
                                      C.c_void_p, C.c_size_t, C.c_void_p]),
    "th_conv_pack_bytes": (C.c_size_t, [C.c_int, C.c_int, C.c_int]),
    "th_conv_pack": (C.c_int, [C.c_void_p, C.c_void_p, C.c_int, C.c_int, C.c_int, C.c_void_p, C.c_size_t,
                               C.POINTER(C.c_float), C.c_void_p]),
    "th_conv2d_supported": (C.c_int, [C.c_int, C.c_int, C.c_int, C.c_int]),
    "th_conv2d": (C.c_int, [C.c_void_p, C.c_void_p, C.c_int, C.c_int, C.c_int, C.c_int, C.c_void_p, C.c_float, C.c_int,
                            C.c_int, C.c_int, C.c_void_p, C.c_void_p]),
    "th_maxpool3x3s2": (C.c_int, [C.c_void_p, C.c_void_p, C.c_int, C.c_int, C.c_int, C.c_void_p, C.c_void_p]),
    "th_bn_workspace_bytes": (C.c_size_t, [C.c_int, C.c_int, C.c_int]),
    "th_bn_act": (C.c_int, [C.c_void_p, C.c_void_p, C.c_void_p, C.c_int, C.c_int, C.c_int, C.c_void_p, C.c_void_p,
                            C.c_float, C.c_float, C.c_void_p, C.c_void_p, C.c_int, C.c_void_p, C.c_void_p, C.c_size_t,
                            C.c_void_p]),
    "th_bn_act_eval": (C.c_int, [C.c_void_p, C.c_void_p, C.c_void_p, C.c_int, C.c_int, C.c_int, C.c_void_p, C.c_void_p,
                                 C.c_float, C.c_void_p, C.c_void_p, C.c_int, C.c_void_p, C.c_void_p]),
    "th_conv2d_stats_partials": (C.c_int, [C.c_int] * 7),
    "th_conv2d_stats": (C.c_int, [C.c_void_p, C.c_void_p, C.c_int, C.c_int, C.c_int, C.c_int, C.c_void_p, C.c_float, C.c_int,
                                  C.c_int, C.c_int, C.c_void_p, C.c_void_p, C.c_size_t, C.c_void_p]),
    "th_bn_act_stats": (C.c_int, [C.c_void_p, C.c_void_p, C.c_void_p, C.c_int, C.c_int, C.c_int, C.c_void_p, C.c_int,
                                  C.c_void_p, C.c_void_p, C.c_float, C.c_float, C.c_void_p, C.c_void_p, C.c_int, C.c_void_p,
                                  C.c_void_p]),
    "th_render_prepass_cancel": (C.c_int, [C.c_void_p]),
    "th_render_prepass_drop": (C.c_int, [C.c_void_p, C.c_void_p]),
    "th_sigma_grid_workspace_bytes": (C.c_size_t, [C.POINTER(ThFrame), C.c_int]),
    "th_eval_sigma_grid": (C.c_int, [C.c_void_p, C.POINTER(ThFrame), C.c_void_p, C.c_int, C.c_void_p, C.c_void_p,
                                     C.c_size_t, C.c_void_p, C.c_size_t, C.POINTER(C.c_int64), C.c_void_p]),
}

_lib = None
_ctx = {}


class HipError(RuntimeError):
    pass


def load_library():
    global _lib
    if _lib is not None:
        return _lib
    if not os.path.exists(LIB_PATH):
        raise HipError(f"{LIB_PATH} not found: build it with `python -m transhuman_amd.build` "
                       "(there is no CPU/torch fallback for the rendering hot path)")
    lib = C.CDLL(LIB_PATH, mode=C.RTLD_GLOBAL)
    for name, (res, args) in SYMBOLS.items():
        fn = getattr(lib, name)
        fn.restype = res
        fn.argtypes = args
    if lib.th_abi_version() != 12:
        raise HipError("ABI version mismatch")
    _lib = lib
    return lib


def _check(rc):
    if rc != 0:
        raise HipError(_lib.th_last_error().decode())


_ctx_by_device = {}
_have_gpu = None


def _gpu_visible():
    global _have_gpu
    if _have_gpu is None:
        _have_gpu = bool(torch.cuda.is_available())
    return _have_gpu


def ctx(device=None):
    h = _ctx_by_device.get(device) if device is not None else None
# ... 939 lines not shown
    lib = load_library()
    d = _f32(ray_d).reshape(-1, 3)
    out = torch.empty((d.shape[0], 3 + 6 * view_res), dtype=torch.float32, device=d.device)
    _check(lib.th_view_embed(ctx(d.device), _p(d), d.shape[0], view_res, _p(out), _stream()))
    return out


class Frame:

    def __init__(self, verts_world, Rh, Th, cams, scale_xy, pixel_map_nhwc, tokens, centres, rot,
                 hull_thresh=0.1, small_frame_rays=2400):
        self.verts = _f32(verts_world).reshape(-1, 3)
        self.Rh, self.Th = _f32(Rh).reshape(9), _f32(Th).reshape(3)
        self.cams, self.scale = cams, scale_xy
        self.map = pixel_map_nhwc
        self.centres, self.rot = _f32(centres).reshape(-1, 3), _f32(rot).reshape(-1, 9)
        self.tokens = _f32(tokens) if tokens is not None else None
        V, H, W, Cc = pixel_map_nhwc.shape
        assert Cc in (384, 260) or isinstance(pixel_map_nhwc, SplitMap), \
            "pixel map must be the full (384) or the compact (260 interleaved / SplitMap) channels-last map"
        src = getattr(pixel_map_nhwc, "source", None)
        self.c = ThFrame(_p(self.verts), self.verts.shape[0], _p(self.Rh), _p(self.Th), _p(self.cams), _p(self.scale),
                         _p(self.map), V, H, W, Cc, _p(self.tokens), _p(self.centres), _p(self.rot),
                         self.centres.shape[0], hull_thresh, small_frame_rays,
                         C.cast(C.pointer(src[0]), C.c_void_p).value if src is not None else None,
                         _p(getattr(pixel_map_nhwc, "fold", None)))

    def set_tokens(self, tokens):
        self.tokens = _f32(tokens)
        assert self.tokens.shape[1] == self.centres.shape[0]
        self.c.tokens = self.tokens.data_ptr()


_ws_cache = {}


def _cached_ws(nbytes, device, slot=0):
    key = (str(device), slot)
    cur = _ws_cache.get(key)
    if cur is None or cur.numel() < nbytes:
        _ws_cache[key] = None
        cur = torch.empty(int(nbytes), dtype=torch.uint8, device=device)
        _ws_cache[key] = cur
    return cur


_pool_cache = {}


def _shade_pool(frame_c, n_valid, with_pregather, device, slot=None):
    need = int(load_library().th_shade_pool_bytes(ctx(device), C.byref(frame_c), int(n_valid), int(with_pregather)))
    key = str(device) if slot is None else (str(device), int(slot))
    cur = _pool_cache.get(key)
    if cur is None or cur.numel() < need:
        _pool_cache[key] = None
        cur = torch.empty(int(need * 1.0625) + 4096, dtype=torch.uint8, device=device)
        _pool_cache[key] = cur
    cur.record_stream(torch.cuda.current_stream(device))
    return cur


def _prepass_counts(ws, device):
    out = (C.c_int64 * 3)()
    rc = load_library().th_render_prepass_wait(ctx(device), _p(ws), out)
    if rc == 1:
        return None
    _check(rc)
    return int(out[0]), int(out[1]), int(out[2])


def drop_workspaces(device=None):
    lib = load_library()
    for key in list(_pool_cache.keys()):
        dev = key if isinstance(key, str) else key[0]
        if device is None or str(device) == dev:
            _pool_cache.pop(key, None)
    for (dev, _slot) in list(_ws_cache.keys()):
        if device is None or str(device) == dev:
            _ws_cache.pop((dev, _slot), None)
    try:
        _check(lib.th_render_prepass_cancel(ctx(device)))
    except HipError:
        pass


def render_prepass(points, verts_world, V, hull_thresh=0.1, small_frame_rays=2400, n_clusters=0, slot=0):
    lib = load_library()
    v = _f32(verts_world).reshape(-1, 3)
    dev = v.device
    f = ThFrame()
    f.verts_world, f.n_verts, f.V = v.data_ptr(), v.shape[0], V
    f.hull_thresh, f.small_frame_rays, f.map_channels = hull_thresh, small_frame_rays, 384
    f.n_clusters = n_clusters
    ws = _cached_ws(lib.th_render_workspace_bytes(C.byref(f), points.R, points.S), dev, slot)
    points._prepass_keep = (v, ws)
    points._prepass_nc = int(n_clusters)
    _check(lib.th_render_prepass(ctx(dev), C.byref(f), C.byref(points.c), _p(ws), ws.numel(), _stream()))
    points._prepass_pending = True


def render_predemand(points, cams, scale_xy, V, H, W, verts_paint=None):
    if not getattr(points, "_prepass_pending", False) or int(W) % 64 != 0 or V > 3:
        return None
    lib = load_library()
    v, ws = points._prepass_keep
    dev = v.device
    f = ThFrame()
    f.verts_world, f.n_verts, f.V, f.H, f.W = v.data_ptr(), v.shape[0], int(V), int(H), int(W)
    f.cams, f.scale_xy = cams.data_ptr(), scale_xy.data_ptr()
    f.n_clusters, f.map_channels = points._prepass_nc, 384
    vp = _f32(verts_paint).reshape(-1, 3) if verts_paint is not None else None
    nb = int(lib.th_map_demand_bytes(int(V), int(H), int(W)))
    demand = torch.empty(nb, dtype=torch.uint8, device=dev)
    rc = lib.th_render_predemand(ctx(dev), C.byref(f), C.byref(points.c), _p(ws), ws.numel(), _p(vp), vp.shape[0] if vp is not None else 0,
                                 _p(demand), nb, _stream())
    if rc == 1:
        return None
    _check(rc)
    demand._keep = (vp, cams, scale_xy)
    return demand


def render_pregrid(frame, points):
    if not getattr(points, "_prepass_pending", False):
        return
    _, ws = points._prepass_keep
    _check(load_library().th_render_pregrid(ctx(frame.verts.device), C.byref(frame.c), C.byref(points.c), _p(ws), ws.numel(),
                                            _stream()))


def render_pregather(net, frame, points, slot=0, early=False, pool_slot=None):
    if not getattr(points, "_prepass_pending", False):
        return
    lib = load_library()
    _sync_weights(net, "mlp")
    dev = frame.verts.device
    _, ws = points._prepass_keep
    cnt = _prepass_counts(ws, dev)
    if cnt is None:
        return
    pool = _shade_pool(frame.c, cnt[2], True, dev, pool_slot)
    points._pregathered = True
    fn = lib.th_render_pregather_early if early else lib.th_render_pregather
    _check(fn(ctx(dev), C.byref(frame.c), C.byref(points.c), _p(ws), ws.numel(), _p(pool), pool.numel(), _stream()))


def render_rays(net, frame, points, white_bkgd=False, defer_guard=False, small_frame_rays=None, pool_slot=None):
    lib = load_library()
    _sync_weights(net, "mlp")
    dev = frame.verts.device
    R = points.R
    rgb = torch.empty((R, 3), dtype=torch.float32, device=dev)
    acc = torch.empty(R, dtype=torch.float32, device=dev)
    dep = torch.empty(R, dtype=torch.float32, device=dev)
    if R == 0:
        st0 = dict(hit_rays=0, valid_samples=0, unmasked=0)
        return (rgb, acc, dep, st0, lambda: True) if defer_guard else (rgb, acc, dep, st0)
    fc = frame.c
    if small_frame_rays is not None and int(small_frame_rays) != fc.small_frame_rays:
        fc = ThFrame.from_buffer_copy(frame.c)
        fc.small_frame_rays = int(small_frame_rays)
    need = lib.th_render_workspace_bytes(C.byref(fc), R, points.S)
    n_bound, pre = R * points.S, False
    if getattr(points, "_prepass_pending", False) and points._prepass_keep[1].numel() >= need:
        points._prepass_pending = False
        ws = points._prepass_keep[1]
# ... 17 lines not shown
            break
        if (conv_fallback(dev) or vit_fallback(dev)) and getattr(frame, "rebuild", None) is not None:
            frame = frame.rebuild()
            keep_sfr = fc.small_frame_rays
            fc = ThFrame.from_buffer_copy(frame.c)
            fc.small_frame_rays = keep_sfr
        _check(lib.th_render_prepass_drop(ctx(dev), _p(ws)))
        pool = _shade_pool(fc, st["valid_samples"], False, dev, pool_slot)
        _check(lib.th_render_rays(ctx(dev), C.byref(fc), C.byref(points.c), _p(rgb), _p(acc), _p(dep),
                                  int(white_bkgd), _p(ws), ws.numel(), _p(pool), pool.numel(), stats, _stream()))
        st = dict(hit_rays=stats[0], valid_samples=stats[1], unmasked=stats[3])
        slot = int(stats[2])
    return rgb, acc, dep, st


def eval_sigma_grid(net, frame, pts):
    lib = load_library()
    _sync_weights(net, "mlp")
    p = _f32(pts).reshape(-1, 3)
    P = p.shape[0]
    out = torch.empty(P, dtype=torch.float32, device=p.device)
    if P == 0:
        return out, dict(valid_samples=0)
    ws = _cached_ws(lib.th_sigma_grid_workspace_bytes(C.byref(frame.c), P), p.device)
    stats = (C.c_int64 * 4)()
    for _ in range(3):
        pool = _shade_pool(frame.c, P, False, p.device)
        _check(lib.th_eval_sigma_grid(ctx(p.device), C.byref(frame.c), _p(p), P, _p(out), _p(ws), ws.numel(), _p(pool),
                                      pool.numel(), stats, _stream()))
        if _guard(p.device, int(stats[2])):
            break
        if (conv_fallback(p.device) or vit_fallback(p.device)) and getattr(frame, "rebuild", None) is not None:
            frame = frame.rebuild()
    return out, dict(valid_samples=stats[1])


def set_tok_gather(on, device=None):
    _check(load_library().th_set_tok_gather(ctx(device), 1 if on else 0))


_tex_rows = {}


def tex_rows_enabled(device=None):
    if _tex_rows:
        d = _dev_index(device)
        if d in _tex_rows:
            return _tex_rows[d]
    return os.environ.get("TH_ROWS_TEX", "1")[:1] != "0"


def mlp_is_fused(device=None):
    d = _dev_index(device)
    return _user_mode.get(d, 1) == 1 and not _range_fallback.get(d)


def set_tex_rows(on, device=None):
    _check(load_library().th_set_tex_rows(ctx(device), 1 if on else 0))
    _tex_rows[_dev_index(device)] = bool(on)


def set_mlp_mode(mode, device=None):
    _check(load_library().th_set_mlp_mode(ctx(device), int(mode)))
    d = _dev_index(device)
    _user_mode[d] = int(mode)
    _range_fallback.pop(d, None)


_fused_waves = {}


def set_fused_waves(waves, device=None):
    _check(load_library().th_set_fused_waves(ctx(device), int(waves)))
    _fused_waves[_dev_index(device)] = int(waves)


def fused_waves(device=None):
    dflt = 4 if os.environ.get("TH_FUSED_WAVES", "8")[:1] == "4" else 8
    if device is None and not torch.cuda.is_available():
        return dflt
    return _fused_waves.get(_dev_index(device), dflt)


def set_chunk_samples(n):
    _check(load_library().th_set_chunk_samples(int(n)))


PROF_PHASES = ("hull", "dparf", "gather", "mlp", "composite", "vit", "fold", "_7")


def profile_enable(on=True, device=None):
    _check(load_library().th_profile_enable(ctx(device), int(on)))


def profile_read(device=None):
    ms = (C.c_double * 8)()
    cnt = (C.c_int64 * 8)()
    _check(load_library().th_profile_read(ctx(device), ms, cnt))
    return {PROF_PHASES[i]: (ms[i], cnt[i]) for i in range(7)}


def clock_probe(out):
    assert out.dtype == torch.int64 and out.numel() >= 3 and out.is_cuda
    _check(load_library().th_clock_probe(ctx(out.device), _p(out), _stream()))


def fused_cycles(counters, device=None):
    if counters is not None:
        assert counters.dtype == torch.int64 and counters.numel() >= 64 and counters.is_cuda
        device = counters.device
    _check(load_library().th_fused_cycles(ctx(device), _p(counters) if counters is not None else None))


def host_wait_read(device=None):
    ms = C.c_double()
    _check(load_library().th_host_wait_read(ctx(device), C.byref(ms)))
    return float(ms.value)


def set_vit_mode(mode, device=None):
    dev = torch.device("cuda", torch.cuda.current_device()) if device is None else torch.device(device)
    _check(load_library().th_set_vit_mode(ctx(dev), int(mode)))
    _vit_graph_epoch[0] += 1
    _user_vit_mode[_dev_index(dev)] = int(mode)
    if int(mode) != 0:
        _vit_fallback.pop(_dev_index(dev), None)
```

Baseline: 19.22 million.

## Add split-phase 8-wave fused MLP variant and peel GEMM pipeline tail

Adds an opt-in SPLIT variant of the 8-wave fused MLP kernel. In it, two half-tile wave groups run the kv/attention/fc layers in opposite phases so that memory and MFMA work overlap, selected via a new context setting (default off). The existing GEMM loops now peel the last iteration, so they no longer issue clamped redundant weight and activation loads at the end of each pipeline. The peeling assumes at least two k-steps. A workspace layout query API is also added.

```diff
diff --git a/include/transhuman_hip.h b/include/transhuman_hip.h
--- a/include/transhuman_hip.h
+++ b/include/transhuman_hip.h
@@ -51,6 +51,8 @@
 int th_set_mlp_weights(th_ctx* ctx, const th_mlp_weights* w, th_stream stream);
 int th_set_mlp_mode(th_ctx* ctx, int mode);
 int th_set_fused_waves(th_ctx* ctx, int waves);
+#define TH_FUSED_SPLIT_DEFAULT 0
+int th_set_fused_split(th_ctx* ctx, int split);
 int th_set_tok_gather(th_ctx* ctx, int on);
 int th_set_tex_rows(th_ctx* ctx, int on);
 
@@ -287,6 +289,7 @@
 } th_frame;
 
 size_t th_render_workspace_bytes(const th_frame* f, int R, int S);
+int th_render_workspace_layout(const th_frame* f, int R, int S, size_t* mask_offset, size_t* raw_offset);
 size_t th_shade_pool_bytes(th_ctx* ctx, const th_frame* f, long long n_valid, int with_pregather);
 int th_render_rays(th_ctx* ctx, const th_frame* f, const th_points* rays, float* rgb, float* acc,
                    float* depth, int white_bkgd, void* workspace, size_t workspace_bytes,
diff --git a/transhuman_amd/csrc/k_mlp_fused8_kernel.h b/transhuman_amd/csrc/k_mlp_fused8_kernel.h
--- a/transhuman_amd/csrc/k_mlp_fused8_kernel.h
+++ b/transhuman_amd/csrc/k_mlp_fused8_kernel.h
@@ -83,27 +83,26 @@
     if (!PRE) f8_load_w<CT>(wl, 0, w[0]);
     f8_load_x<NR, ROWSTEP, PERM>(ahi, alo, aoff, 0, xah, xal);
     FM_SB();
-    auto step = [&](auto first, auto par, int t) __attribute__((always_inline)) {
-        constexpr bool F = decltype(first)::value;
+    auto step = [&](auto first, auto last, auto par, int t) __attribute__((always_inline)) {
+        constexpr bool F = decltype(first)::value, L = decltype(last)::value;
         constexpr int PB = decltype(par)::value;
-        const int tn = t + 1 < T ? t + 1 : T - 1;
         f8_load_x<NR, ROWSTEP, PERM>(ahi + NR * ROWSTEP, alo + NR * ROWSTEP, aoff, t, xbh, xbl);
-        f8_load_w<CT>(wl, tn, w[PB ^ 1]);
+        if constexpr (!L) f8_load_w<CT>(wl, t + 1, w[PB ^ 1]);
         f8_mfma_half<CT, RT, NR, 0, F>(w[PB], xah, xal, acc);
-        f8_interleave<2 * NR + 2 * CT, 3 * CT * NR>();
-        f8_load_x<NR, ROWSTEP, PERM>(ahi, alo, aoff, tn, xah, xal);
+        f8_interleave<2 * NR + (L ? 0 : 2 * CT), 3 * CT * NR>();
+        if constexpr (!L) f8_load_x<NR, ROWSTEP, PERM>(ahi, alo, aoff, t + 1, xah, xal);
         f8_mfma_half<CT, RT, NR, NR, F>(w[PB], xbh, xbl, acc);
-        f8_interleave<2 * NR, 3 * CT * NR>();
+        f8_interleave<(L ? 0 : 2 * NR), 3 * CT * NR>();
     };
-    step(std::true_type{}, std::integral_constant<int, 0>{}, 0);
-    if (T > 1) {
-        step(std::false_type{}, std::integral_constant<int, 1>{}, 1);
+    step(std::true_type{}, std::false_type{}, std::integral_constant<int, 0>{}, 0);
+    step(std::false_type{}, std::false_type{}, std::integral_constant<int, 1>{}, 1);
 #pragma unroll 1
-        for (int t = 2; t < T; t += 2) {
-            step(std::false_type{}, std::integral_constant<int, 0>{}, t);
-            step(std::false_type{}, std::integral_constant<int, 1>{}, t + 1);
-        }
-    }
+    for (int t = 2; t < T - 2; t += 2) {
+        step(std::false_type{}, std::false_type{}, std::integral_constant<int, 0>{}, t);
+        step(std::false_type{}, std::false_type{}, std::integral_constant<int, 1>{}, t + 1);
+    }
+    step(std::false_type{}, std::false_type{}, std::integral_constant<int, 0>{}, T - 2);
+    step(std::false_type{}, std::true_type{}, std::integral_constant<int, 1>{}, T - 1);
 }
 
 template <int RT, int CT, int ROWSTEP, bool PERM, bool PRE = false>
@@ -117,25 +116,28 @@
     if (!PRE) f8_load_w<CT>(wl, 0, w[0]);
     f8_load_x<NR, ROWSTEP, PERM>(ahi, alo, aoff, 0, xh[0], xl[0]);
     FM_SB();
-    auto sub = [&](auto first, auto sidx, int t) __attribute__((always_inline)) {
+    auto sub = [&](auto first, auto last, auto sidx, int t) __attribute__((always_inline)) {
         constexpr int S = decltype(sidx)::value, G = S % 3, PB = S / 3, CUR = S & 1;
         constexpr bool F = decltype(first)::value && S < 3;
+        constexpr bool END = decltype(last)::value && PB == 1;
         constexpr int GN = (G + 1) % 3;
+        constexpr bool LDX = !(END && G == 2), LDW = G == 0 && !END;
         const int tt = t + PB;
-        const int tx = G == 2 ? (tt + 1 < T ? tt + 1 : T - 1) : tt;
-        f8_load_x<NR, ROWSTEP, PERM>(ahi + GN * NR * ROWSTEP, alo + GN * NR * ROWSTEP, aoff, tx, xh[CUR ^ 1], xl[CUR ^ 1]);
-        if constexpr (G == 0) f8_load_w<CT>(wl, tt + 1 < T ? tt + 1 : T - 1, w[PB ^ 1]);
+        const int tx = G == 2 ? tt + 1 : tt;
+        if constexpr (LDX) f8_load_x<NR, ROWSTEP, PERM>(ahi + GN * NR * ROWSTEP, alo + GN * NR * ROWSTEP, aoff, tx, xh[CUR ^ 1], xl[CUR ^ 1]);
+        if constexpr (LDW) f8_load_w<CT>(wl, tt + 1, w[PB ^ 1]);
         f8_mfma_half<CT, RT, NR, G * NR, F>(w[PB], xh[CUR], xl[CUR], acc);
-        f8_interleave<2 * NR + (G == 0 ? 2 * CT : 0), 3 * CT * NR>();
+        f8_interleave<(LDX ? 2 * NR : 0) + (LDW ? 2 * CT : 0), 3 * CT * NR>();
     };
-    auto pair = [&](auto first, int t) __attribute__((always_inline)) {
-        sub(first, std::integral_constant<int, 0>{}, t); sub(first, std::integral_constant<int, 1>{}, t);
-        sub(first, std::integral_constant<int, 2>{}, t); sub(first, std::integral_constant<int, 3>{}, t);
-        sub(first, std::integral_constant<int, 4>{}, t); sub(first, std::integral_constant<int, 5>{}, t);
+    auto pair = [&](auto first, auto last, int t) __attribute__((always_inline)) {
+        sub(first, last, std::integral_constant<int, 0>{}, t); sub(first, last, std::integral_constant<int, 1>{}, t);
+        sub(first, last, std::integral_constant<int, 2>{}, t); sub(first, last, std::integral_constant<int, 3>{}, t);
+        sub(first, last, std::integral_constant<int, 4>{}, t); sub(first, last, std::integral_constant<int, 5>{}, t);
     };
-    pair(std::true_type{}, 0);
+    pair(std::true_type{}, std::false_type{}, 0);
 #pragma unroll 1
-    for (int t = 2; t < T; t += 2) pair(std::false_type{}, t);
+    for (int t = 2; t < T - 2; t += 2) pair(std::false_type{}, std::false_type{}, t);
+    pair(std::false_type{}, std::true_type{}, T - 2);
 }
 template <int RT, int CT, int ROWSTEP, bool PERM, bool PRE = false>
 __device__ __forceinline__ void f8_gemm_rt(const char* __restrict__ ahi, const char* __restrict__ alo, int str,
@@ -191,7 +193,9 @@
     }
 }
 
-template <int V>
+#include "k_mlp_fused8_split.h"
+
+template <int V, bool SPLIT = false>
 __global__ __launch_bounds__(F8_THREADS, 2) void mlp_fused8_kernel(FusedParams P_arg) {
 #define PK P_arg
     struct F8Dbg { long long* dbg; };
@@ -533,6 +537,304 @@
         }
         range_commit(PK.range, TH_RANGE_S, seen_s, rmax);
     }
+    char* vd_hi = mbuf + MBUF_VD_OFF;
+    char* vd_lo = vd_hi + 32 * STRVD;
+    f8_f4 va[1][RT];
+    if constexpr (SPLIT) {
+        const int grp = __builtin_amdgcn_readfirstlane(wave >> 2), wq = __builtin_amdgcn_readfirstlane(wave & 3);
+        const int ltid = tid & 255;
+        const int row0 = grp * 16 + l15;
+        const char* gh = abuf + grp * RS256;
+        const char* gl = a256_lo + grp * RS256;
+        float* ksb = reinterpret_cast<float*>(mbuf);
+        float* kpb = reinterpret_cast<float*>(abuf);
+        static_assert(KSTR * 4 == STR256, "a key row overlays one hi-plane row");
+        constexpr std::integral_constant<int, 0> c0{};
+        constexpr std::integral_constant<int, 1> c1{};
+        uint4 wk3[2][3][2];
+        auto kv_pass = [&](const FusedLayer& L16, const FusedLayer& L, auto sc, int ba, int bb, f8_f4 (&kk)[V], f8_f4 (&vv)[2][V])
+                           __attribute__((always_inline)) {
+            constexpr int S = decltype(sc)::value;
+            const int ow = 2 * wq + S;
+            f8_f4 acc3[3][V];
+            f8s_gemm<V, 3, true, S == 0>(gh, gl, F8_WSLICE(L16, ow, 3), F8_WSLICE(L16, ow + 1, 3), lane, acc3, wk3, ba, bb);
+            const float4 bk = f8_bias(L.bias, ow * 16, lane), bv0 = f8_bias(L.bias, 128 + ow * 32, lane),
+                         bv1 = f8_bias(L.bias, 128 + ow * 32 + 16, lane);
+#pragma unroll
+            for (int v = 0; v < V; ++v) {
+                kk[v] = f8_finish(acc3[0][v], bk, L.inv_scale, false);
+                vv[0][v] = f8_finish(acc3[1][v], bv0, L.inv_scale, false);
+                vv[1][v] = f8_finish(acc3[2][v], bv1, L.inv_scale, false);
+            }
+        };
+        auto keys_out = [&](float* kb, int s, const f8_f4 (&kk)[V]) __attribute__((always_inline)) {
+#pragma unroll
+            for (int v = 0; v < V; ++v)
+                *reinterpret_cast<float4*>(kb + (v * 32 + row0) * KSTR + (2 * wq + s) * 16 + 4 * g4) = make_float4(kk[v][0], kk[v][1], kk[v][2], kk[v][3]);
+        };
+        FM_SB();
+        f8_load_w<3>(F8_WSLICE(PK.w16.kv1, 2 * wq, 3) + lane, 0, wk3[0]);
+        FM_SYNCL();
+        f8_f4 vs[2][2][V];
+        {
+            f8_f4 kk[V];
+            kv_pass(PK.w16.kv1, PK.kv1, c0, -1, -1, kk, vs[0]);
+            keys_out(ksb, 0, kk);
+            kv_pass(PK.w16.kv1, PK.kv1, c1, -1, -1, kk, vs[1]);
+            keys_out(ksb, 1, kk);
+        }
+        FM_SYNCL();
+        FM_SB();
+        fill_tex(tex_pre, std::false_type{}, [] {});
+        FM_SB();
+        f8_load_w<3>(F8_WSLICE(PK.w16.kv0, 2 * wq, 3) + lane, 0, wk3[0]);
+        if (tid == 0) *flag = 0;
+        FM_SYNCL();
+        if (grp == 1) __builtin_amdgcn_s_barrier();
+        f8_f4 kp[2][V], vp[2][2][V];
+        kv_pass(PK.w16.kv0, PK.kv0, c0, grp == 1 ? 2 : -1, grp == 1 ? 6 : -1, kp[0], vp[0]);
+        kv_pass(PK.w16.kv0, PK.kv0, c1, -1, -1, kp[1], vp[1]);
+        FM_SYNCL();
+        keys_out(kpb, 0, kp[0]);
+        keys_out(kpb, 1, kp[1]);
+        FM_SYNCL();
+        float4 bn[2][2];
+        {
+            const int p = grp * 16 + (ltid >> 4), c16 = ltid & 15;
+            f32x2 sc2[V * V];
+#pragma unroll
+            for (int ji = 0; ji < V * V; ++ji) sc2[ji] = (f32x2){0.f, 0.f};
+#pragma unroll
+            for (int q = 0; q < 2; ++q) {
+                float4 kx[V], sx[V];
+#pragma unroll
+                for (int v = 0; v < V; ++v) {
+                    kx[v] = *reinterpret_cast<const float4*>(kpb + (v * 32 + p) * KSTR + 4 * (c16 + 16 * q));
+                    sx[v] = *reinterpret_cast<const float4*>(ksb + (v * 32 + p) * KSTR + 4 * (c16 + 16 * q));
+                }
+#pragma unroll
+                for (int j = 0; j < V; ++j)
+#pragma unroll
+                    for (int i = 0; i < V; ++i) {
+                        sc2[j * V + i] = __builtin_elementwise_fma((f32x2){kx[j].x, kx[j].y}, (f32x2){sx[i].x, sx[i].y}, sc2[j * V + i]);
+                        sc2[j * V + i] = __builtin_elementwise_fma((f32x2){kx[j].z, kx[j].w}, (f32x2){sx[i].z, sx[i].w}, sc2[j * V + i]);
+                    }
+            }
+            float acc[V * V];
+#pragma unroll
+            for (int ji = 0; ji < V * V; ++ji) {
+                float s = sc2[ji][0] + sc2[ji][1];
+                s += __builtin_bit_cast(float, __builtin_amdgcn_update_dpp(0, __builtin_bit_cast(int, s), 0xB1, 0xF, 0xF, true));
+                s += __builtin_bit_cast(float, __builtin_amdgcn_update_dpp(0, __builtin_bit_cast(int, s), 0x4E, 0xF, 0xF, true));
+                s += __builtin_bit_cast(float, __builtin_amdgcn_update_dpp(0, __builtin_bit_cast(int, s), 0x141, 0xF, 0xF, true));
+                s += __builtin_bit_cast(float, __builtin_amdgcn_update_dpp(0, __builtin_bit_cast(int, s), 0x140, 0xF, 0xF, true));
+                acc[ji] = s;
+            }
+            float a[V], m = -3.0e38f;
+#pragma unroll
+            for (int j = 0; j < V; ++j) {
+                float x = acc[j * V];
+#pragma unroll
+                for (int i = 1; i < V; ++i) x = c16 == i ? acc[j * V + i] : x;
+                a[j] = x / 11.313708498984761f;
+                m = fmaxf(m, a[j]);
+            }
+            float e[V], se = 0.f;
+#pragma unroll
+            for (int j = 0; j < V; ++j) { e[j] = expf(a[j] - m); se = se + e[j]; }
+            if (c16 < V) {
+#pragma unroll
+                for (int j = 0; j < V; ++j) probs[p * F8_PSTR + j * V + c16] = e[j] / se;
+            }
+        }
+#pragma unroll
+        for (int s = 0; s < 2; ++s) {
+            bn[s][0] = f8_bias(PK.fc_1.bias, (2 * wq + s) * 32, lane);
+            bn[s][1] = f8_bias(PK.fc_1.bias, (2 * wq + s) * 32 + 16, lane);
+        }
+        FM_SYNCL();
+        {
+            const float* pr = probs + row0 * F8_PSTR;
+            const float4 q0 = *reinterpret_cast<const float4*>(pr), q1 = *reinterpret_cast<const float4*>(pr + 4);
+            const float q2 = pr[8];
+            const float A[9] = {q0.x, q0.y, q0.z, q0.w, q1.x, q1.y, q1.z, q1.w, q2};
+#pragma unroll
+            for (int s = 0; s < 2; ++s)
+#pragma unroll
+                for (int c = 0; c < 2; ++c) {
+                    const f32x2 b01 = {bn[s][c].x, bn[s][c].y}, b23 = {bn[s][c].z, bn[s][c].w};
+                    f32x2 t0[V], t1[V];
+#pragma unroll
+                    for (int i = 0; i < V; ++i) {
+                        t0[i] = (f32x2){vs[s][c][i][0], vs[s][c][i][1]} + b01;
+                        t1[i] = (f32x2){vs[s][c][i][2], vs[s][c][i][3]} + b23;
+                    }
+#pragma unroll
+                    for (int j = 0; j < V; ++j) {
+                        const f32x2 v0 = {vp[s][c][j][0], vp[s][c][j][1]}, v1 = {vp[s][c][j][2], vp[s][c][j][3]};
+#pragma unroll
+                        for (int i = 0; i < V; ++i) {
+                            const f32x2 a2 = {A[j * V + i], A[j * V + i]};
+                            t0[i] = __builtin_elementwise_fma(v0, a2, t0[i]);
+                            t1[i] = __builtin_elementwise_fma(v1, a2, t1[i]);
+                        }
+                    }
+#pragma unroll
+                    for (int i = 0; i < V; ++i) {
+                        t0[i] = __builtin_elementwise_max(t0[i], (f32x2){0.f, 0.f});
+                        t1[i] = __builtin_elementwise_max(t1[i], (f32x2){0.f, 0.f});
+                        const f8_f4 n = {t0[i][0], t0[i][1], t1[i][0], t1[i][1]};
+                        f8_store_h<STR256>(n, i * 32 + row0, (2 * wq + s) * 32 + c * 16, abuf, a256_lo, lane, rmax);
+                    }
+                }
+            range_commit(PK.range, TH_RANGE_N, seen_n, rmax);
+        }
+        uint4 wk2[2][2][2];
+        FM_SB();
+        f8_load_w<2>(F8_WSLICE(PK.w16.fc_2, 2 * wq, 2) + lane, 0, wk2[0]);
+#pragma unroll
+        for (int q = 0; q < 2; ++q) {
+            const int i = tid + F8_THREADS * q, row = i >> 5, c = i & 31;
+            int x = pbase + row;
+            if (PK.vd_sel != nullptr && PK.rgb_all != 2 && c < 27 && row < npts) x = PK.vd_sel[pbase + row];
+            vsel[q] = x;
+        }
+        FM_SYNCL();
+        f8_f4 ai[2][2][V];
+        f8s_gemm<V, 2, true, true>(gh, gl, F8_WSLICE(PK.w16.fc_2, 2 * wq, 2), F8_WSLICE(PK.w16.fc_2, 2 * wq + 1, 2), lane, ai[0], wk2,
+                                   grp == 0 ? 2 : -1, -1);
+        f8s_gemm<V, 2, true, false>(gh, gl, F8_WSLICE(PK.w16.fc_2, 2 * wq + 1, 2), nullptr, lane, ai[1], wk2, grp == 0 ? 2 : -1, -1);
+        float4 bi[2][2];
+#pragma unroll
+        for (int s = 0; s < 2; ++s) {
+            bi[s][0] = f8_bias(PK.fc_2.bias, (2 * wq + s) * 32, lane);
+            bi[s][1] = f8_bias(PK.fc_2.bias, (2 * wq + s) * 32 + 16, lane);
+        }
+#pragma unroll
+        for (int q = 0; q < 2; ++q) {
+            const int i = tid + F8_THREADS * q, row = i >> 5, c = i & 31;
+            float x = 0.f;
+            if (PK.rgb_all != 2 && c < 27 && row < npts) {
+                const long long vr = PK.vd_sel ? (long long)(vsel[q] / PK.vd_div) : (long long)(pbase + row);
+                x = PK.vd[vr * 27 + c];
+            }
+            vdv[q] = x;
+        }
+        FM_SYNCL();
+#pragma unroll
+        for (int s = 0; s < 2; ++s)
+#pragma unroll
+            for (int c = 0; c < 2; ++c) {
+                const int col = (2 * wq + s) * 32 + c * 16;
+#pragma unroll
+                for (int v = 0; v < V; ++v) ai[s][c][v] = f8_finish(ai[s][c][v], bi[s][c], PK.fc_2.inv_scale, true);
+                f8_f4 m = ai[s][c][0];
+#pragma unroll
+                for (int v = 1; v < V; ++v) m = m + ai[s][c][v];
+                m = m * (f8_f4){inv_v, inv_v, inv_v, inv_v};
+                f8_store_h<STR256>(m, row0, col, mbuf, mbuf + 32 * STR256, lane, rmax);
+#pragma unroll
+                for (int v = 0; v < V; ++v) f8_store_h<STR256>(ai[s][c][v], v * 32 + row0, col, abuf, a256_lo, lane, rmax);
+            }
+        range_commit(PK.range, TH_RANGE_INTER, seen_i, rmax);
+        FM_SYNCL();
+        tex_pre2 = tex_fetch();
+        f8_f4 a3[2][2][2], vas[2][1][V];
+        float4 aw[2][2], b3[2][2];
+#pragma unroll
+        for (int s = 0; s < 2; ++s)
+#pragma unroll
+            for (int c = 0; c < 2; ++c) {
+                aw[s][c] = f8_bias(PK.alpha_w, (2 * wq + s) * 32 + c * 16, lane);
+                b3[s][c] = f8_bias(PK.fc_3.bias, (2 * wq + s) * 32 + c * 16, lane);
+            }
+        {
+            const char* mhi = mbuf + grp * RS256;
+            const char* mlo = mbuf + 32 * STR256 + grp * RS256;
+            const uint4* w3a = F8_WSLICE(PK.w16.fc_3, 2 * wq, 2);
+            const uint4* w3b = F8_WSLICE(PK.w16.fc_3, 2 * wq + 1, 2);
+            if (PK.rgb_all != 2) {
+                const uint4* waa = F8_WSLICE(PK.w16.vfA, 2 * wq, 1);
+                const uint4* wab = F8_WSLICE(PK.w16.vfA, 2 * wq + 1, 1);
+                uint4 r3[2][2][2], ra[2][1][2];
+                f8s_dual<V, true>(mhi, mlo, gh, gl, w3a, waa, w3b, wab, lane, a3[0], vas[0], r3, ra, false, grp == 1 ? 2 : -1);
+                f8s_dual<V, false>(mhi, mlo, gh, gl, w3b, wab, nullptr, nullptr, lane, a3[1], vas[1], r3, ra, true, -1);
+            } else {
+                uint4 w3[2][2][2];
+                f8_f4 a1[2][2][1];
+                f8s_gemm<1, 2, false, true>(mhi, mlo, w3a, w3b, lane, a1[0], w3, grp == 1 ? 2 : -1, -1);
+                f8s_gemm<1, 2, true, false>(mhi, mlo, w3b, nullptr, lane, a1[1], w3, -1, -1);
+#pragma unroll
+                for (int s = 0; s < 2; ++s) {
+                    a3[s][0][0] = a1[s][0][0];
+                    a3[s][1][0] = a1[s][1][0];
+#pragma unroll
+                    for (int v = 0; v < V; ++v) vas[s][0][v] = (f8_f4){0.f, 0.f, 0.f, 0.f};
+                }
+            }
+        }
+        FM_SYNCL();
+        {
+            float s2[2];
+#pragma unroll
+            for (int s = 0; s < 2; ++s) {
+                float sm = 0.f;
+#pragma unroll
+                for (int c = 0; c < 2; ++c) {
+                    const f8_f4 y = f8_finish(a3[s][c][0], b3[s][c], PK.fc_3.inv_scale, true);
+                    sm = fmaf(y[0], aw[s][c].x, sm);
+                    sm = fmaf(y[1], aw[s][c].y, sm);
+                    sm = fmaf(y[2], aw[s][c].z, sm);
+                    sm = fmaf(y[3], aw[s][c].w, sm);
+                }
+                sm += f8_xor(sm, lane, 16);
+                sm += f8_xor(sm, lane, 32);
+                s2[s] = sm;
+            }
+            if (g4 == 0) part[(2 * wq) * 32 + row0] = s2[0];
+            if (g4 == 1) part[(2 * wq + 1) * 32 + row0] = s2[1];
+        }
+        FM_SYNCL();
+        if (ltid < 16) {
+            const int smp = grp * 16 + ltid;
+            float sg = PK.alpha_b[zoff];
+#pragma unroll
+            for (int w = 0; w < 8; ++w) sg += part[w * 32 + smp];
+            sig[smp] = sg;
+            if (smp < npts && PK.rgb_all != 2 && (PK.rgb_all == 1 || sg > 0.f)) *flag = 1;
+        }
+        FM_SYNCL();
+        if (grp == 0) {
+            FM_SYNCL();
+            FM_SYNCL();
+        }
+#pragma unroll
+        for (int q = 0; q < 2; ++q) {
+            const int i = tid + F8_THREADS * q, row = i >> 5, c = i & 31;
+            _Float16 a, b;
+            split_h(vdv[q], a, b);
+            *reinterpret_cast<_Float16*>(vd_hi + row * STRVD + 2 * c) = a;
+            *reinterpret_cast<_Float16*>(vd_lo + row * STRVD + 2 * c) = b;
+        }
+        {
+            f8_f4* xb = reinterpret_cast<f8_f4*>(abuf);
+            static_assert(8 * 2 * V * 64 * 16 <= ABUF_BYTES, "the view_fc hand-back must fit the operand buffer");
+#pragma unroll
+            for (int s = 0; s < 2; ++s)
+#pragma unroll
+                for (int v = 0; v < V; ++v) xb[(((2 * wq + s) * 2 + grp) * V + v) * 64 + lane] = vas[s][0][v];
+        }
+        FM_SYNCL();
+        if (*flag != 0) {
+            const f8_f4* xb = reinterpret_cast<const f8_f4*>(abuf);
+#pragma unroll
+            for (int r = 0; r < RT; ++r) va[0][r] = xb[((wave * 2 + (r & 1)) * V + (r >> 1)) * 64 + lane];
+            FM_SYNCL();
+        } else {
+#pragma unroll
+            for (int r = 0; r < RT; ++r) va[0][r] = (f8_f4){0.f, 0.f, 0.f, 0.f};
+        }
+    } else {
     uint4 wk3[2][3][2];
     FM_SB();
     f8_load_w<3>(F8_WSLICE(PK.w16.kv1, wave, 3) + lane, 0, wk3[0]);
@@ -710,10 +1012,7 @@
     range_commit(PK.range, TH_RANGE_INTER, seen_i, rmax);
     FM_SYNCL();
 
-    char* vd_hi = mbuf + MBUF_VD_OFF;
-    char* vd_lo = vd_hi + 32 * STRVD;
     tex_pre2 = tex_fetch();
-    f8_f4 va[1][RT];
     {
         f8_f4 a3[2][2];
         const float4 aw[2] = {f8_bias(PK.alpha_w, wave * 32, lane), f8_bias(PK.alpha_w, wave * 32 + 16, lane)};
@@ -732,28 +1031,33 @@
             f8_load_x<1, RS256, true>(mhi, mlo, aoff, 0, mah, mal);
             f8_load_x<V, RS256, true>(abuf, a256_lo, aoff, 0, xah, xal);
             FM_SB();
-            auto step = [&](auto first, auto par, int t) __attribute__((always_inline)) {
-                constexpr bool F = decltype(first)::value;
+            auto step = [&](auto first, auto last, auto par, int t) __attribute__((always_inline)) {
+                constexpr bool F = decltype(first)::value, L = decltype(last)::value;
                 constexpr int PB = decltype(par)::value;
-                const int tn = t + 1 < T ? t + 1 : T - 1;
                 f8_load_x<1, RS256, true>(mhi + RS256, mlo + RS256, aoff, t, mbh, mbl);
                 f8_load_x<V, RS256, true>(abuf + V * RS256, a256_lo + V * RS256, aoff, t, xbh, xbl);
-                f8_load_w<2>(w3l, tn, r3[PB ^ 1]);
-                f8_load_w<1>(wal, tn, ra[PB ^ 1]);
+                if constexpr (!L) {
+                    f8_load_w<2>(w3l, t + 1, r3[PB ^ 1]);
+                    f8_load_w<1>(wal, t + 1, ra[PB ^ 1]);
+                }
                 f8_mfma_dual<RT, V, 0, 0, F>(r3[PB], ra[PB], mah, mal, xah, xal, a3, va);
-                f8_interleave<2 + 2 * V + 6, 3 * (2 + V)>();
-                f8_load_x<1, RS256, true>(mhi, mlo, aoff, tn, mah, mal);
-                f8_load_x<V, RS256, true>(abuf, a256_lo, aoff, tn, xah, xal);
+                f8_interleave<2 + 2 * V + (L ? 0 : 6), 3 * (2 + V)>();
+                if constexpr (!L) {
+                    f8_load_x<1, RS256, true>(mhi, mlo, aoff, t + 1, mah, mal);
+                    f8_load_x<V, RS256, true>(abuf, a256_lo, aoff, t + 1, xah, xal);
+                }
                 f8_mfma_dual<RT, V, 1, V, F>(r3[PB], ra[PB], mbh, mbl, xbh, xbl, a3, va);
-                f8_interleave<2 + 2 * V, 3 * (2 + V)>();
+                f8_interleave<(L ? 0 : 2 + 2 * V), 3 * (2 + V)>();
             };
-            step(std::true_type{}, std::integral_constant<int, 0>{}, 0);
-            step(std::false_type{}, std::integral_constant<int, 1>{}, 1);
+            step(std::true_type{}, std::false_type{}, std::integral_constant<int, 0>{}, 0);
+            step(std::false_type{}, std::false_type{}, std::integral_constant<int, 1>{}, 1);
 #pragma unroll 1
-            for (int t = 2; t < T; t += 2) {
-                step(std::false_type{}, std::integral_constant<int, 0>{}, t);
-                step(std::false_type{}, std::integral_constant<int, 1>{}, t + 1);
-            }
+            for (int t = 2; t < T - 2; t += 2) {
+                step(std::false_type{}, std::false_type{}, std::integral_constant<int, 0>{}, t);
+                step(std::false_type{}, std::false_type{}, std::integral_constant<int, 1>{}, t + 1);
+            }
+            step(std::false_type{}, std::false_type{}, std::integral_constant<int, 0>{}, T - 2);
+            step(std::false_type{}, std::true_type{}, std::integral_constant<int, 1>{}, T - 1);
         } else {
 #pragma unroll
             for (int r = 0; r < RT; ++r) va[0][r] = (f8_f4){0.f, 0.f, 0.f, 0.f};
@@ -796,6 +1100,7 @@
             *reinterpret_cast<_Float16*>(vd_lo + row * STRVD + 2 * c) = b;
         }
         FM_SYNCL();
+    }
     }
     const bool need_rgb = *flag != 0;
     float rgb_out[3] = {0.f, 0.f, 0.f};
diff --git a/transhuman_amd/csrc/k_mlp_fused8_split.h b/transhuman_amd/csrc/k_mlp_fused8_split.h
--- /dev/null
+++ b/transhuman_amd/csrc/k_mlp_fused8_split.h
@@ -0,0 +1,98 @@
+#pragma once
+#include <utility>
+
+#define F8S_ROWSTEP (32 * STR256)
+
+__device__ __forceinline__ void f8s_absorb(int t, int ba, int bb) {
+    if (t == ba) __builtin_amdgcn_s_barrier();
+    if (t == bb) __builtin_amdgcn_s_barrier();
+}
+template <int... S, class FN>
+__device__ __forceinline__ void f8s_each(std::integer_sequence<int, S...>, FN&& fn) {
+    (fn(std::integral_constant<int, S>{}), ...);
+}
+
+template <int NV, int CT, bool PRE, bool NEXT>
+__device__ __forceinline__ void f8s_gemm(const char* __restrict__ ahi, const char* __restrict__ alo, const uint4* __restrict__ wp,
+                                         const uint4* __restrict__ wnext, int lane, f8_f4 (&acc)[CT][NV], uint4 (&w)[2][CT][2],
+                                         int ba, int bb) {
+    constexpr int T = 8;
+    const uint4* wl = wp + lane;
+    const int aoff = f8_aoff<true>(lane, STR256);
+    h8 xh[2][1], xl[2][1];
+    if (!PRE) f8_load_w<CT>(wl, 0, w[0]);
+    f8_load_x<1, F8S_ROWSTEP, true>(ahi, alo, aoff, 0, xh[0], xl[0]);
+    FM_SB();
+    auto sub = [&](auto first, auto last, auto sidx, int t) __attribute__((always_inline)) {
+        constexpr int S = decltype(sidx)::value, G = S % NV, PB = S / NV, CUR = S & 1;
+        constexpr bool F = decltype(first)::value && S < NV;
+        constexpr bool END = decltype(last)::value && PB == 1;
+        constexpr int GN = (G + 1) % NV;
+        constexpr bool WRAP = G == NV - 1;
+        constexpr bool LDX = !(END && WRAP), LDW = G == 0 && !END, LDN = NEXT && END && G == 0;
+        const int tt = t + PB;
+        if constexpr (LDX)
+            f8_load_x<1, F8S_ROWSTEP, true>(ahi + GN * F8S_ROWSTEP, alo + GN * F8S_ROWSTEP, aoff, WRAP ? tt + 1 : tt, xh[CUR ^ 1], xl[CUR ^ 1]);
+        if constexpr (LDW) f8_load_w<CT>(wl, tt + 1, w[PB ^ 1]);
+        if constexpr (LDN) f8_load_w<CT>(wnext + lane, 0, w[0]);
+        f8_mfma_half<CT, NV, 1, G, F>(w[PB], xh[CUR], xl[CUR], acc);
+        f8_interleave<(LDX ? 2 : 0) + (LDW || LDN ? 2 * CT : 0), 3 * CT>();
+    };
+    auto pair = [&](auto first, auto last, int t) __attribute__((always_inline)) {
+        f8s_each(std::make_integer_sequence<int, 2 * NV>{}, [&](auto s) __attribute__((always_inline)) { sub(first, last, s, t); });
+    };
+    pair(std::true_type{}, std::false_type{}, 0);
+#pragma unroll 1
+    for (int t = 2; t < T - 2; t += 2) {
+        f8s_absorb(t, ba, bb);
+        pair(std::false_type{}, std::false_type{}, t);
+    }
+    f8s_absorb(T - 2, ba, bb);
+    pair(std::false_type{}, std::true_type{}, T - 2);
+}
+
+template <int NV, bool NEXT>
+__device__ __forceinline__ void f8s_dual(const char* __restrict__ mhi, const char* __restrict__ mlo, const char* __restrict__ xhi,
+                                         const char* __restrict__ xlo, const uint4* __restrict__ w3p, const uint4* __restrict__ wap,
+                                         const uint4* __restrict__ w3next, const uint4* __restrict__ wanext, int lane,
+                                         f8_f4 (&a3)[2][2], f8_f4 (&va)[1][NV], uint4 (&r3)[2][2][2], uint4 (&ra)[2][1][2], bool pre,
+                                         int ba) {
+    constexpr int T = 8;
+    const uint4* w3l = w3p + lane;
+    const uint4* wal = wap + lane;
+    const int aoff = f8_aoff<true>(lane, STR256);
+    h8 mh[2][1], ml[2][1], xh[2][NV], xl[2][NV];
+    if (!pre) {
+        f8_load_w<2>(w3l, 0, r3[0]);
+        f8_load_w<1>(wal, 0, ra[0]);
+    }
+    f8_load_x<1, F8S_ROWSTEP, true>(mhi, mlo, aoff, 0, mh[0], ml[0]);
+    f8_load_x<NV, F8S_ROWSTEP, true>(xhi, xlo, aoff, 0, xh[0], xl[0]);
+    FM_SB();
+    auto step = [&](auto first, auto last, auto par, int t) __attribute__((always_inline)) {
+        constexpr bool F = decltype(first)::value, L = decltype(last)::value;
+        constexpr int PB = decltype(par)::value;
+        if constexpr (!L) {
+            f8_load_x<1, F8S_ROWSTEP, true>(mhi, mlo, aoff, t + 1, mh[PB ^ 1], ml[PB ^ 1]);
+            f8_load_x<NV, F8S_ROWSTEP, true>(xhi, xlo, aoff, t + 1, xh[PB ^ 1], xl[PB ^ 1]);
+            f8_load_w<2>(w3l, t + 1, r3[PB ^ 1]);
+            f8_load_w<1>(wal, t + 1, ra[PB ^ 1]);
+        } else if constexpr (NEXT) {
+            f8_load_w<2>(w3next + lane, 0, r3[0]);
+            f8_load_w<1>(wanext + lane, 0, ra[0]);
+        }
+        f8_mfma_dual<NV, NV, 0, 0, F>(r3[PB], ra[PB], mh[PB], ml[PB], xh[PB], xl[PB], a3, va);
+        f8_interleave<(L ? (NEXT ? 6 : 0) : 2 + 2 * NV + 6), 3 * (2 + NV)>();
+    };
+    step(std::true_type{}, std::false_type{}, std::integral_constant<int, 0>{}, 0);
+    step(std::false_type{}, std::false_type{}, std::integral_constant<int, 1>{}, 1);
+#pragma unroll 1
+    for (int t = 2; t < T - 2; t += 2) {
+        f8s_absorb(t, ba, -1);
+        step(std::false_type{}, std::false_type{}, std::integral_constant<int, 0>{}, t);
+        step(std::false_type{}, std::false_type{}, std::integral_constant<int, 1>{}, t + 1);
+    }
+    f8s_absorb(T - 2, ba, -1);
+    step(std::false_type{}, std::false_type{}, std::integral_constant<int, 0>{}, T - 2);
+    step(std::false_type{}, std::true_type{}, std::integral_constant<int, 1>{}, T - 1);
+}
diff --git a/transhuman_amd/csrc/k_mlp_fused_host.hip b/transhuman_amd/csrc/k_mlp_fused_host.hip
--- a/transhuman_amd/csrc/k_mlp_fused_host.hip
+++ b/transhuman_amd/csrc/k_mlp_fused_host.hip
@@ -415,6 +415,9 @@
         TH_HIP(hipFuncSetAttribute((const void*)mlp_fused8_kernel<1>, hipFuncAttributeMaxDynamicSharedMemorySize, F8_LDS_BYTES));
         TH_HIP(hipFuncSetAttribute((const void*)mlp_fused8_kernel<2>, hipFuncAttributeMaxDynamicSharedMemorySize, F8_LDS_BYTES));
         TH_HIP(hipFuncSetAttribute((const void*)mlp_fused8_kernel<3>, hipFuncAttributeMaxDynamicSharedMemorySize, F8_LDS_BYTES));
+        TH_HIP(hipFuncSetAttribute((const void*)mlp_fused8_kernel<1, true>, hipFuncAttributeMaxDynamicSharedMemorySize, F8_LDS_BYTES));
+        TH_HIP(hipFuncSetAttribute((const void*)mlp_fused8_kernel<2, true>, hipFuncAttributeMaxDynamicSharedMemorySize, F8_LDS_BYTES));
+        TH_HIP(hipFuncSetAttribute((const void*)mlp_fused8_kernel<3, true>, hipFuncAttributeMaxDynamicSharedMemorySize, F8_LDS_BYTES));
     }
     static int dbg_state = getenv("TH_FUSED_DBG") ? 1 : 0;
     static long long* dbg_dev = nullptr;
@@ -433,7 +436,10 @@
 #define FM_LAUNCH(V_, F_) hipLaunchKernelGGL((mlp_fused_kernel<V_, F_>), grid, dim3(256), FUSED_LDS_BYTES, s, p)
 #define FM_LAUNCH_T(V_) hipLaunchKernelGGL((mlp_fused_kernel<V_, 1, true>), grid, dim3(256), FUSED_LDS_BYTES, s, p)
 #define FM_LAUNCH_8(V_) hipLaunchKernelGGL((mlp_fused8_kernel<V_>), grid, dim3(F8_THREADS), F8_LDS_BYTES, s, p)
-    if (eight) {
+#define FM_LAUNCH_8S(V_) hipLaunchKernelGGL((mlp_fused8_kernel<V_, true>), grid, dim3(F8_THREADS), F8_LDS_BYTES, s, p)
+    if (eight && base.split != 0) {
+        if (V == 1) FM_LAUNCH_8S(1); else if (V == 2) FM_LAUNCH_8S(2); else FM_LAUNCH_8S(3);
+    } else if (eight) {
         if (V == 1) FM_LAUNCH_8(1); else if (V == 2) FM_LAUNCH_8(2); else FM_LAUNCH_8(3);
     } else if (tex) {
         if (V == 1) FM_LAUNCH_T(1); else if (V == 2) FM_LAUNCH_T(2); else FM_LAUNCH_T(3);
@@ -449,6 +455,7 @@
 #undef FM_LAUNCH
 #undef FM_LAUNCH_T
 #undef FM_LAUNCH_8
+#undef FM_LAUNCH_8S
     TH_LAUNCH_CHECK();
     if (dbg_now) {
         long long st[64];
diff --git a/transhuman_amd/csrc/th_api.hip b/transhuman_amd/csrc/th_api.hip
--- a/transhuman_amd/csrc/th_api.hip
+++ b/transhuman_amd/csrc/th_api.hip
@@ -79,6 +79,8 @@
     if (const char* e = getenv("TH_ROWS_TEX")) c->tex_rows = e[0] == '0' ? 0 : 1;
     c->fused.waves = 8;
     if (const char* e = getenv("TH_FUSED_WAVES")) c->fused.waves = e[0] == '4' ? 4 : 8;
+    c->fused.split = TH_FUSED_SPLIT_DEFAULT;
+    if (const char* e = getenv("TH_FUSED_SPLIT")) c->fused.split = e[0] == '1' ? 1 : 0;
     TH_HIP(hipHostMalloc((void**)&c->host_pinned, 64 * sizeof(int32_t), hipHostMallocDefault));
     TH_HIP(hipMalloc((void**)&c->range_dev, TH_RANGE_SLOTS * sizeof(unsigned int)));
     TH_HIP(hipMemset(c->range_dev, 0, TH_RANGE_SLOTS * sizeof(unsigned int)));
@@ -327,6 +329,11 @@
 int th_set_fused_waves(th_ctx* c, int waves) {
     TH_REQUIRE(c && (waves == 4 || waves == 8), "th_set_fused_waves: 4 (one wave per SIMD) or 8 (two per SIMD)");
     c->fused.waves = waves;
+    return 0;
+}
+int th_set_fused_split(th_ctx* c, int split) {
+    TH_REQUIRE(c && (split == 0 || split == 1), "th_set_fused_split: 0 (lock-step) or 1 (half tiles in opposite phases)");
+    c->fused.split = split;
     return 0;
 }
 
@@ -1253,6 +1260,16 @@
     return shade_ws_bytes(f, (long long)R * S, R);
 }
 
+int th_render_workspace_layout(const th_frame* f, int R, int S, size_t* mask_offset, size_t* raw_offset) {
+    TH_REQUIRE(f && R >= 1 && S >= 1 && mask_offset && raw_offset, "bad argument");
+    char* const origin = reinterpret_cast<char*>((size_t)256);
+    ThArena ar(origin, ~(size_t)0 >> 2);
+    const ShadeWs w = carve_shade_ws(f, (long long)R * S, R, ar);
+    *mask_offset = (size_t)(reinterpret_cast<char*>(w.mask) - origin);
+    *raw_offset = (size_t)(reinterpret_cast<char*>(w.raw) - origin);
+    return 0;
+}
+
 size_t th_shade_pool_bytes(th_ctx* c, const th_frame* f, long long n_valid, int with_pregather) {
     if (!c || !f || f->V < 1) return 0;
     const int f_ld = frame_f_ld(f);
diff --git a/transhuman_amd/csrc/th_internal.h b/transhuman_amd/csrc/th_internal.h
--- a/transhuman_amd/csrc/th_internal.h
+++ b/transhuman_amd/csrc/th_internal.h
@@ -217,6 +217,7 @@
 struct FusedParams {
     Fused16 w16;
     int waves;
+    int split;
     FusedLayer fc_0pe;
     FusedLayer kv1, ar0, kv0, fc_1, fc_2, fc_3, fc_4;
     FusedLayer vfA, vfD, rst;
diff --git a/transhuman_amd/hip.py b/transhuman_amd/hip.py
--- a/transhuman_amd/hip.py
+++ b/transhuman_amd/hip.py
@@ -62,6 +62,7 @@
     "th_set_mlp_weights": (C.c_int, [C.c_void_p, C.POINTER(ThMlpWeights), C.c_void_p]),
     "th_set_mlp_mode": (C.c_int, [C.c_void_p, C.c_int]),
     "th_set_fused_waves": (C.c_int, [C.c_void_p, C.c_int]),
+    "th_set_fused_split": (C.c_int, [C.c_void_p, C.c_int]),
     "th_set_vit_mode": (C.c_int, [C.c_void_p, C.c_int]),
     "th_set_tok_gather": (C.c_int, [C.c_void_p, C.c_int]),
     "th_set_tex_rows": (C.c_int, [C.c_void_p, C.c_int]),
@@ -173,6 +174,7 @@
                               C.c_void_p, C.c_void_p, C.c_void_p, C.c_size_t, C.c_void_p]),
     "th_view_embed": (C.c_int, [C.c_void_p, C.c_void_p, C.c_int, C.c_int, C.c_void_p, C.c_void_p]),
     "th_render_workspace_bytes": (C.c_size_t, [C.POINTER(ThFrame), C.c_int, C.c_int]),
+    "th_render_workspace_layout": (C.c_int, [C.POINTER(ThFrame), C.c_int, C.c_int, C.POINTER(C.c_size_t), C.POINTER(C.c_size_t)]),
     "th_shade_pool_bytes": (C.c_size_t, [C.c_void_p, C.POINTER(ThFrame), C.c_longlong, C.c_int]),
     "th_render_prepass_wait": (C.c_int, [C.c_void_p, C.c_void_p, C.POINTER(C.c_int64)]),
     "th_render_rays": (C.c_int, [C.c_void_p, C.POINTER(ThFrame), C.POINTER(ThPoints), C.c_void_p, C.c_void_p,
@@ -1278,6 +1280,12 @@
         _check(lib.th_render_prepass_cancel(ctx(device)))
     except HipError:
         pass
+
+
+def render_workspace_layout(frame, R, S):
+    m, r = C.c_size_t(0), C.c_size_t(0)
+    _check(load_library().th_render_workspace_layout(C.byref(frame.c), int(R), int(S), C.byref(m), C.byref(r)))
+    return int(m.value), int(r.value)
 
 
 def render_prepass(points, verts_world, V, hull_thresh=0.1, small_frame_rays=2400, n_clusters=0, slot=0):
@@ -1461,6 +1469,23 @@
     return _fused_waves.get(_dev_index(device), dflt)
 
 
+_fused_split = {}
+FUSED_SPLIT_DEFAULT = 0
+
+
+def set_fused_split(split, device=None):
+    _check(load_library().th_set_fused_split(ctx(device), int(split)))
+    _fused_split[_dev_index(device)] = int(split)
+
+
+def fused_split(device=None):
+    e = os.environ.get("TH_FUSED_SPLIT")
+    dflt = FUSED_SPLIT_DEFAULT if e is None else (1 if e[:1] == "1" else 0)
+    if device is None and not torch.cuda.is_available():
+        return dflt
+    return _fused_split.get(_dev_index(device), dflt)
+
+
 def set_chunk_samples(n):
     _check(load_library().th_set_chunk_samples(int(n)))
 
```

Measured after the change: 19.36 million, median of 6. Within noise of the previous version (+0.7%).
